# tensorflow/adanet

Hardware: AMD Instinct MI355X
Metric: adanet_iterations_per_hour (higher is better)
Workload: dtype bf16; 1 GPU; model=cifar10-dnn-search (adanet paper space), global_batch=2048, input_dim=3072, n_classes=10, hidden=2048, candidates_per_iter=2, train_steps_per_iter=150, eval_batches=8, parallelism=round_robin1, final_ensemble_size=12

## Files before the change

### adanet_amd/csrc/binding.cpp

```cpp

#include <torch/extension.h>

void gemm_nt_bf16(const at::Tensor& A, const at::Tensor& B, at::Tensor& C,
                  const c10::optional<at::Tensor>& bias, int64_t act,
                  double dropout_p, const c10::optional<at::Tensor>& seed);
void gemm_nt_bf16_probe(const at::Tensor& A, const at::Tensor& B,
                        at::Tensor& C, int64_t variant);
void gemm_nt8(const at::Tensor& A, const at::Tensor& B, at::Tensor& C,
              const c10::optional<at::Tensor>& bias, int64_t act,
              int64_t variant);
void gemm_x8(const at::Tensor& A, const at::Tensor& B, at::Tensor& C,
             const c10::optional<at::Tensor>& bias, int64_t act,
             int64_t trans_a, int64_t trans_b, int64_t variant);
void probe_tr16_layout(at::Tensor& out);
void gemm_tr_probe(const at::Tensor& A, const at::Tensor& B, at::Tensor& C,
                   int64_t trans_a, int64_t trans_b, int64_t variant);
void gemm_tr_bf16(const at::Tensor& A, const at::Tensor& B, at::Tensor& C,
                  const c10::optional<at::Tensor>& bias, int64_t act,
                  int64_t trans_a, int64_t trans_b);
void gemm_tr_batched(const at::Tensor& A, const at::Tensor& B, at::Tensor& C,
                     const c10::optional<at::Tensor>& bias, int64_t act,
                     int64_t trans_a, int64_t trans_b);
void transpose_bf16(const at::Tensor& in, at::Tensor& out);
void softmax_xent_fwd(const at::Tensor& logits, const at::Tensor& labels,
                      const c10::optional<at::Tensor>& loss,
                      at::Tensor& probs, double eps,
                      const c10::optional<at::Tensor>& mean_out);
void softmax_xent_bwd(const at::Tensor& probs, const at::Tensor& labels,
                      const c10::optional<at::Tensor>& grad_rows,
                      at::Tensor& dlogits, double eps,
                      const c10::optional<at::Tensor>& grad_scalar);
void mixer_bwd_dlogits(const at::Tensor& dY, const at::Tensor& weights,
                       at::Tensor& dL, int64_t j, int64_t vector_mode);
void mixer_fwd_direct(const std::vector<at::Tensor>& members,
                      const at::Tensor& weights,
                      const c10::optional<at::Tensor>& bias, at::Tensor& out,
                      int64_t vector_mode);
void mixer_bwd_dw_direct(const std::vector<at::Tensor>& members,
                         const at::Tensor& dY, at::Tensor& dw,
                         int64_t vector_mode);
void fused_sgd(at::Tensor& master, at::Tensor& param, const at::Tensor& grad,
               const c10::optional<at::Tensor>& momentum_buf, double lr,
               double momentum, double dampening, double weight_decay,
               bool nesterov, double grad_scale);
void fused_adam(at::Tensor& master, at::Tensor& param, const at::Tensor& grad,
                at::Tensor& m_buf, at::Tensor& v_buf, double lr, double beta1,
                double beta2, double eps, double weight_decay, int64_t step,
                double grad_scale);
void fused_sgd_fp32(at::Tensor& param, const at::Tensor& grad,
                    const c10::optional<at::Tensor>& momentum_buf, double lr,
                    double momentum, double dampening, double weight_decay,
                    bool nesterov, double grad_scale);
void fused_adam_fp32(at::Tensor& param, const at::Tensor& grad,
                     at::Tensor& m_buf, at::Tensor& v_buf, double lr,
                     double beta1, double beta2, double eps,
                     double weight_decay, int64_t step, double grad_scale);
void layernorm_fwd(const at::Tensor& x, const c10::optional<at::Tensor>& gamma,
                   const c10::optional<at::Tensor>& beta, at::Tensor& y,
                   at::Tensor& mean, at::Tensor& rstd, double eps);
void layernorm_bwd(const at::Tensor& x, const at::Tensor& dy,
                   const c10::optional<at::Tensor>& gamma,
                   const at::Tensor& mean, const at::Tensor& rstd,
                   at::Tensor& dx, const c10::optional<at::Tensor>& dgamma,
                   const c10::optional<at::Tensor>& dbeta);
void dropout_fwd(const at::Tensor& x, at::Tensor& y, double p,
                 const at::Tensor& seed);
void dropout_bwd(const at::Tensor& dy, at::Tensor& dx, double p,
                 const at::Tensor& seed);
void relu_bwd(const at::Tensor& dy, const at::Tensor& y, at::Tensor& dx,
              double scale);
void relu_bwd_colsum(const at::Tensor& dy, const at::Tensor& y,
                     at::Tensor& dz, at::Tensor& db, double scale);
void multi_copy_bf16(const std::vector<at::Tensor>& srcs,
                     const std::vector<at::Tensor>& dsts);
void cell_combine_fwd(const std::vector<at::Tensor>& lefts,
                      const std::vector<at::Tensor>& rights,
                      const std::vector<at::Tensor>& scales_l,
                      const std::vector<at::Tensor>& scales_r, at::Tensor& out,
                      int64_t block_offset);
void cell_combine_bwd(const at::Tensor& dy,
                      const std::vector<at::Tensor>& scales_l,
                      const std::vector<at::Tensor>& scales_r,
                      const std::vector<c10::optional<at::Tensor>>& dlefts,
                      const std::vector<c10::optional<at::Tensor>>& drights,
                      int64_t block_offset);
void augment_draw(const at::Tensor& labels, at::Tensor& params,
                  at::Tensor& labels_out, uint64_t seed, int64_t step,
                  int64_t rank, int64_t world, int64_t N, int64_t pad,
                  int64_t H, int64_t W, bool augment);
void augment_apply(const at::Tensor& data, const at::Tensor& params,
                   const at::Tensor& scale, const at::Tensor& shift,
                   at::Tensor& out, int64_t pad, int64_t cutout_pad);
void colsum_bf16(const at::Tensor& x, at::Tensor& out, int64_t accum);
void binary_histogram(const at::Tensor& scores, const at::Tensor& labels,
                      at::Tensor& hist);
void metrics_multiclass_update(at::Tensor& state, const at::Tensor& logits,
                               const at::Tensor& labels, int64_t k,
                               double eps, bool per_class);
void metrics_binary_update(at::Tensor& state, const at::Tensor& logits,
                           const at::Tensor& labels, int64_t T);
void metrics_regression_update(at::Tensor& state, const at::Tensor& logits,
                               const at::Tensor& labels);
int64_t metrics_max_blocks();
void depthwise_fwd(const at::Tensor& x, const at::Tensor& w, at::Tensor& y,
                   int64_t stride, int64_t pad);
void depthwise_bwd_dx(const at::Tensor& dy, const at::Tensor& w,
                      at::Tensor& dx, int64_t stride, int64_t pad);
void depthwise_bwd_dw(const at::Tensor& x, const at::Tensor& dy,
                      at::Tensor& dw, int64_t stride, int64_t pad);
void argmax_correct(const at::Tensor& logits, const at::Tensor& labels,
                    const c10::optional<at::Tensor>& pred, at::Tensor& correct);
void im2col_bf16(const at::Tensor& x, at::Tensor& out, int64_t K,
                 int64_t stride, int64_t pad);
void col2im_bf16(const at::Tensor& du, at::Tensor& dx, int64_t K,
                 int64_t stride, int64_t pad);
void pool3_fwd(const at::Tensor& x, at::Tensor& y,
               const c10::optional<at::Tensor>& argmax, int64_t stride,
               int64_t is_max);
void pool3_bwd(const at::Tensor& dy, const c10::optional<at::Tensor>& argmax,
               at::Tensor& dx, int64_t stride, int64_t is_max);
void batchnorm_stats(const at::Tensor& x, at::Tensor& mean, at::Tensor& rstd,
                     const c10::optional<at::Tensor>& running_mean,
                     const c10::optional<at::Tensor>& running_var,
                     double eps, double momentum);
void batchnorm_norm(const at::Tensor& x, at::Tensor& y,
                    const at::Tensor& mean, const at::Tensor& rstd,
                    const c10::optional<at::Tensor>& gamma,
                    const c10::optional<at::Tensor>& beta);
void batchnorm_bwd(const at::Tensor& x, const at::Tensor& dy, at::Tensor& dx,
                   const at::Tensor& mean, const at::Tensor& rstd,
                   const c10::optional<at::Tensor>& gamma, at::Tensor& sdy,
                   at::Tensor& sdyx);

PYBIND11_MODULE(TORCH_EXTENSION_NAME, m) {
  m.doc() = "adanet_amd gfx950 (MI355X/CDNA4) kernels";
  m.def("gemm_nt_bf16", &gemm_nt_bf16,
        "C[M,N] = A[M,K] @ B[N,K]^T, fused bias/relu/dropout",
        py::arg("A"), py::arg("B"), py::arg("C"), py::arg("bias"),
        py::arg("act"), py::arg("dropout_p") = 0.0,
        py::arg("seed") = c10::nullopt);
  m.def("gemm_nt_bf16_probe", &gemm_nt_bf16_probe);
  m.def("gemm_nt8", &gemm_nt8,
        "8-phase deep-pipelined GEMM (256^2-class tiles)");
  m.def("gemm_x8", &gemm_x8,
        "pipelined GEMM with K-major (transposed) operand staging");
  m.def("probe_tr16_layout", &probe_tr16_layout);
  m.def("gemm_tr_probe", &gemm_tr_probe);
  m.def("gemm_tr_bf16", &gemm_tr_bf16);
  m.def("gemm_tr_batched", &gemm_tr_batched);
  m.def("transpose_bf16", &transpose_bf16, "bf16 2-D transpose");
  m.def("softmax_xent_fwd", &softmax_xent_fwd);
  m.def("softmax_xent_bwd", &softmax_xent_bwd);
  m.def("mixer_bwd_dlogits", &mixer_bwd_dlogits);
  m.def("mixer_fwd_direct", &mixer_fwd_direct);
  m.def("mixer_bwd_dw_direct", &mixer_bwd_dw_direct);
  m.def("fused_sgd", &fused_sgd);
  m.def("fused_adam", &fused_adam);
  m.def("fused_sgd_fp32", &fused_sgd_fp32);
  m.def("fused_adam_fp32", &fused_adam_fp32);
  m.def("layernorm_fwd", &layernorm_fwd);
  m.def("layernorm_bwd", &layernorm_bwd);
  m.def("dropout_fwd", &dropout_fwd);
  m.def("dropout_bwd", &dropout_bwd);
  m.def("relu_bwd", &relu_bwd, py::arg("dy"), py::arg("y"), py::arg("dx"),
        py::arg("scale") = 1.0);
  m.def("relu_bwd_colsum", &relu_bwd_colsum, py::arg("dy"), py::arg("y"),
        py::arg("dz"), py::arg("db"), py::arg("scale") = 1.0);
  m.def("multi_copy_bf16", &multi_copy_bf16);
  m.def("cell_combine_fwd", &cell_combine_fwd,
        "fused drop-path scale + add + channel concat of up to 8 block pairs",
        py::arg("lefts"), py::arg("rights"), py::arg("scales_l"),
        py::arg("scales_r"), py::arg("out"), py::arg("block_offset") = 0);
  m.def("cell_combine_bwd", &cell_combine_bwd, py::arg("dy"),
        py::arg("scales_l"), py::arg("scales_r"), py::arg("dlefts"),
        py::arg("drights"), py::arg("block_offset") = 0);
  m.def("augment_draw", &augment_draw,
        "per-sample (index, oy, ox, flip, cy, cx) from the counter RNG, plus "
        "the gathered labels",
        py::arg("labels"), py::arg("params"), py::arg("labels_out"),
        py::arg("seed"), py::arg("step"), py::arg("rank"), py::arg("world"),
        py::arg("N"), py::arg("pad"), py::arg("H"), py::arg("W"),
        py::arg("augment") = true);
  m.def("augment_apply", &augment_apply,
        "fused gather + pad-crop + flip + cutout + normalise + bf16 cast",
        py::arg("data"), py::arg("params"), py::arg("scale"),
        py::arg("shift"), py::arg("out"), py::arg("pad"),
        py::arg("cutout_pad"));
  m.def("colsum_bf16", &colsum_bf16, py::arg("x"), py::arg("out"),
        py::arg("accum") = 0);
  m.def("argmax_correct", &argmax_correct);
  m.def("binary_histogram", &binary_histogram);
  m.def("metrics_multiclass_update", &metrics_multiclass_update,
        "streaming loss / top-1 / top-k / per-class counts into an fp64 state",
        py::arg("state"), py::arg("logits"), py::arg("labels"), py::arg("k"),
        py::arg("eps"), py::arg("per_class"));
  m.def("metrics_binary_update", &metrics_binary_update,
        "streaming sigmoid loss / accuracy / [2,T] score histogram",
        py::arg("state"), py::arg("logits"), py::arg("labels"), py::arg("T"));
  m.def("metrics_regression_update", &metrics_regression_update,
        "streaming squared / absolute error sums", py::arg("state"),
        py::arg("logits"), py::arg("labels"));
  m.def("metrics_max_blocks", &metrics_max_blocks,
        "grid cap of the streaming-metric update kernels");
  m.def("im2col_bf16", &im2col_bf16);
  m.def("col2im_bf16", &col2im_bf16);
  m.def("pool3_fwd", &pool3_fwd);
  m.def("pool3_bwd", &pool3_bwd);
  m.def("batchnorm_stats", &batchnorm_stats);
  m.def("batchnorm_norm", &batchnorm_norm);
  m.def("batchnorm_bwd", &batchnorm_bwd);
  m.def("depthwise_fwd", &depthwise_fwd);
  m.def("depthwise_bwd_dx", &depthwise_bwd_dx);
  m.def("depthwise_bwd_dw", &depthwise_bwd_dw);
}
```

### adanet_amd/csrc/common.h

```cpp
#pragma once

#include <hip/hip_runtime.h>
#include <hip/hip_bf16.h>
#include <cstdint>

#define WAVE 64

using bf16_t = __hip_bfloat16;

typedef __attribute__((ext_vector_type(4))) float f32x4;
typedef __attribute__((ext_vector_type(8))) short s16x8;
typedef __attribute__((ext_vector_type(4))) short s16x4;
typedef __attribute__((ext_vector_type(2))) short s16x2;
typedef __attribute__((ext_vector_type(4))) int i32x4;

__device__ __forceinline__ float bf2f(bf16_t x) { return __bfloat162float(x); }
__device__ __forceinline__ bf16_t f2bf(float x) { return __float2bfloat16(x); }

__device__ __forceinline__ float bits2f(short s) {
  union { unsigned int u; float f; } cvt;
  cvt.u = ((unsigned int)(unsigned short)s) << 16;
  return cvt.f;
}

__device__ __forceinline__ short f2bits(float f) {
  union { unsigned int u; float f; } cvt;
  cvt.f = f;
  unsigned int u = cvt.u;
  unsigned int rounding = 0x7fff + ((u >> 16) & 1);
  return (short)((u + rounding) >> 16);
}

__device__ __forceinline__ float wave_reduce_sum(float v) {
#pragma unroll
  for (int off = 32; off > 0; off >>= 1) v += __shfl_xor(v, off, 64);
  return v;
}

__device__ __forceinline__ float wave_reduce_max(float v) {
#pragma unroll
  for (int off = 32; off > 0; off >>= 1) v = fmaxf(v, __shfl_xor(v, off, 64));
  return v;
}


template <int N, typename Emit>
__device__ __forceinline__ void block_reduce_sum(const float (&acc)[N],
                                                 Emit emit) {
  __shared__ float partial[4];
#pragma unroll
  for (int t = 0; t < N; ++t) {
    const float v = wave_reduce_sum(acc[t]);
    if ((threadIdx.x & 63) == 0) partial[threadIdx.x >> 6] = v;
    __syncthreads();
    if (threadIdx.x == 0)
      emit(t, partial[0] + partial[1] + partial[2] + partial[3]);
    __syncthreads();
  }
}

__device__ __forceinline__ float wave_slot_sum(const float* __restrict__ base,
                                               int64_t stride, int n) {
  float s = 0.f;
  for (int r = threadIdx.x & 63; r < n; r += 64) s += base[r * stride];
  return wave_reduce_sum(s);
}

void launch_colsum_reduce(const float* wsp, float* out, int C, int nchunks,
                          int accum, hipStream_t stream);

__device__ __forceinline__ uint32_t hash_rng(uint64_t seed, uint64_t idx) {
  uint64_t z = seed + 0x9e3779b97f4a7c15ull * (idx + 1);
  z = (z ^ (z >> 30)) * 0xbf58476d1ce4e5b9ull;
  z = (z ^ (z >> 27)) * 0x94d049bb133111ebull;
  return (uint32_t)(z >> 32);
}

#define HIP_CHECK_KERNEL()                                                    \
  do {                                                                        \
    hipError_t e = hipGetLastError();                                         \
    if (e != hipSuccess) {                                                    \
      TORCH_CHECK(false, "HIP kernel launch failed: ", hipGetErrorString(e)); \
    }                                                                         \
  } while (0)
```

### adanet_amd/csrc/elementwise.hip

```cpp

#include <torch/extension.h>
#include <ATen/cuda/CUDAContext.h>
#include "common.h"

__global__ __launch_bounds__(256) void dropout_fwd_kernel(
    const bf16_t* __restrict__ x, bf16_t* __restrict__ y, int64_t n, float p,
    const uint64_t* __restrict__ seed_ptr) {
  const float scale = 1.f / (1.f - p);
  const uint32_t thresh = (uint32_t)(p * 4294967296.0f);
  const uint64_t seed = *seed_ptr;
  const int64_t stride = (int64_t)gridDim.x * blockDim.x;
  for (int64_t i = (int64_t)blockIdx.x * blockDim.x + threadIdx.x; i < n;
       i += stride) {
    const bool drop = hash_rng(seed, (uint64_t)i) < thresh;
    y[i] = drop ? f2bf(0.f) : f2bf(bf2f(x[i]) * scale);
  }
}

__global__ __launch_bounds__(256) void dropout_bwd_kernel(
    const bf16_t* __restrict__ dy, bf16_t* __restrict__ dx, int64_t n, float p,
    const uint64_t* __restrict__ seed_ptr) {
  const float scale = 1.f / (1.f - p);
  const uint32_t thresh = (uint32_t)(p * 4294967296.0f);
  const uint64_t seed = *seed_ptr;
  const int64_t stride = (int64_t)gridDim.x * blockDim.x;
  for (int64_t i = (int64_t)blockIdx.x * blockDim.x + threadIdx.x; i < n;
       i += stride) {
    const bool drop = hash_rng(seed, (uint64_t)i) < thresh;
    dx[i] = drop ? f2bf(0.f) : f2bf(bf2f(dy[i]) * scale);
  }
}

__global__ __launch_bounds__(256) void relu_bwd_kernel(
    const bf16_t* __restrict__ dy, const bf16_t* __restrict__ y,
    bf16_t* __restrict__ dx, int64_t n, float scale) {
  const int64_t stride = (int64_t)gridDim.x * blockDim.x;
  for (int64_t i = (int64_t)blockIdx.x * blockDim.x + threadIdx.x; i < n;
       i += stride) {
    dx[i] = bf2f(y[i]) > 0.f ? f2bf(bf2f(dy[i]) * scale) : f2bf(0.f);
  }
}

__global__ __launch_bounds__(256) void relu_bwd_colsum_kernel(
    const bf16_t* __restrict__ dy, const bf16_t* __restrict__ y,
    bf16_t* __restrict__ dz, float* __restrict__ wsp, int B, int C,
    int rows_per_block, float scale) {
  const int c = blockIdx.x * blockDim.x + threadIdx.x;
  if (c >= C) return;
  const int r0 = blockIdx.y * rows_per_block;
  const int r1 = min(B, r0 + rows_per_block);
  float acc = 0.f;
  for (int b = r0; b < r1; ++b) {
    const int64_t i = (int64_t)b * C + c;
    const float g = bf2f(y[i]) > 0.f ? bf2f(dy[i]) * scale : 0.f;
    dz[i] = f2bf(g);
    acc += g;
  }
  wsp[(int64_t)blockIdx.y * C + c] = acc;
}

struct CopyPtrs {
  const bf16_t* s[8];
  bf16_t* d[8];
  int64_t n[8];
};

typedef __attribute__((ext_vector_type(4))) unsigned int u32x4_c;

__global__ __launch_bounds__(256) void multi_copy_bf16_kernel(CopyPtrs P,
                                                              int npairs) {
  const int seg = blockIdx.y;
  if (seg >= npairs) return;
  const bf16_t* __restrict__ s = P.s[seg];
  bf16_t* __restrict__ d = P.d[seg];
  const int64_t n = P.n[seg];
  const int64_t stride = (int64_t)gridDim.x * blockDim.x * 8;
  for (int64_t i = ((int64_t)blockIdx.x * blockDim.x + threadIdx.x) * 8;
       i < n; i += stride) {
    if (i + 8 <= n) {
      *(u32x4_c*)(d + i) = *(const u32x4_c*)(s + i);
    } else {
      for (int64_t j = i; j < n; ++j) d[j] = s[j];
    }
  }
}

void multi_copy_bf16(const std::vector<at::Tensor>& srcs,
                     const std::vector<at::Tensor>& dsts) {
  TORCH_CHECK(srcs.size() == dsts.size(), "multi_copy: pair count mismatch");
  auto stream = at::cuda::getCurrentCUDAStream();
  for (size_t j0 = 0; j0 < srcs.size(); j0 += 8) {
    const int np = (int)std::min<size_t>(8, srcs.size() - j0);
    CopyPtrs P;
    int64_t maxn = 0;
    for (int k = 0; k < np; ++k) {
      const at::Tensor& s = srcs[j0 + k];
      const at::Tensor& d = dsts[j0 + k];
      TORCH_CHECK(s.is_cuda() && d.is_cuda() &&
                      s.scalar_type() == at::kBFloat16 &&
                      d.scalar_type() == at::kBFloat16 &&
                      s.is_contiguous() && d.is_contiguous() &&
                      s.numel() == d.numel(),
                  "multi_copy: contiguous bf16 same-size pairs required");
      P.s[k] = (const bf16_t*)s.data_ptr();
      P.d[k] = (bf16_t*)d.data_ptr();
      P.n[k] = s.numel();
      maxn = std::max(maxn, P.n[k]);
    }
    if (maxn == 0) continue;
    const int blocks =
        (int)std::min<int64_t>((maxn + 8 * 256 - 1) / (8 * 256), 512);
    hipLaunchKernelGGL(multi_copy_bf16_kernel,
                       dim3((unsigned)blocks, (unsigned)np), dim3(256), 0,
                       stream.stream(), P, np);
    HIP_CHECK_KERNEL();
  }
}

static int ew_grid(int64_t n) {
  return (int)std::min<int64_t>((n + 255) / 256, 2048);
}

void dropout_fwd(const at::Tensor& x, at::Tensor& y, double p,
                 const at::Tensor& seed) {
  const int64_t n = x.numel();
  if (n == 0) return;
  TORCH_CHECK(seed.is_cuda() && seed.scalar_type() == at::kLong,
              "dropout: device int64 seed tensor required");
  auto stream = at::cuda::getCurrentCUDAStream();
  hipLaunchKernelGGL(dropout_fwd_kernel, dim3(ew_grid(n)), dim3(256), 0,
                     stream.stream(), (const bf16_t*)x.data_ptr(),
                     (bf16_t*)y.data_ptr(), n, (float)p,
                     (const uint64_t*)seed.data_ptr());
  HIP_CHECK_KERNEL();
}

void dropout_bwd(const at::Tensor& dy, at::Tensor& dx, double p,
                 const at::Tensor& seed) {
  const int64_t n = dy.numel();
  if (n == 0) return;
  auto stream = at::cuda::getCurrentCUDAStream();
  hipLaunchKernelGGL(dropout_bwd_kernel, dim3(ew_grid(n)), dim3(256), 0,
                     stream.stream(), (const bf16_t*)dy.data_ptr(),
                     (bf16_t*)dx.data_ptr(), n, (float)p,
                     (const uint64_t*)seed.data_ptr());
  HIP_CHECK_KERNEL();
}

void relu_bwd(const at::Tensor& dy, const at::Tensor& y, at::Tensor& dx,
              double scale) {
  const int64_t n = dy.numel();
  if (n == 0) return;
  auto stream = at::cuda::getCurrentCUDAStream();
  hipLaunchKernelGGL(relu_bwd_kernel, dim3(ew_grid(n)), dim3(256), 0,
                     stream.stream(), (const bf16_t*)dy.data_ptr(),
                     (const bf16_t*)y.data_ptr(), (bf16_t*)dx.data_ptr(), n,
                     (float)scale);
  HIP_CHECK_KERNEL();
}

void relu_bwd_colsum(const at::Tensor& dy, const at::Tensor& y,
                     at::Tensor& dz, at::Tensor& db, double scale) {
  TORCH_CHECK(dy.is_contiguous() && y.is_contiguous() && dz.is_contiguous(),
              "relu_bwd_colsum: contiguous tensors required");
  TORCH_CHECK(db.scalar_type() == at::kFloat, "relu_bwd_colsum: fp32 db");
  const int B = (int)dy.size(0), C = (int)dy.size(1);
  if (B == 0 || C == 0) return;
  auto stream = at::cuda::getCurrentCUDAStream();
  const int stripes = (C + 255) / 256;
  const int row_chunks =
      std::max(1, std::min(1024 / stripes, (B + 7) / 8));
  const int rows_per_block = (B + row_chunks - 1) / row_chunks;
  auto wsp = at::empty({row_chunks, C}, db.options());
  hipLaunchKernelGGL(relu_bwd_colsum_kernel,
                     dim3((unsigned)stripes, (unsigned)row_chunks), dim3(256),
                     0, stream.stream(), (const bf16_t*)dy.data_ptr(),
                     (const bf16_t*)y.data_ptr(), (bf16_t*)dz.data_ptr(),
                     wsp.data_ptr<float>(), B, C, rows_per_block,
                     (float)scale);
  launch_colsum_reduce(wsp.data_ptr<float>(), db.data_ptr<float>(), C,
                       row_chunks, 1, stream.stream());
  HIP_CHECK_KERNEL();
}
```

### adanet_amd/csrc/gemm_8ph.hip

```cpp

#include <torch/extension.h>
#include <ATen/cuda/CUDAContext.h>
#include "common.h"

namespace {

template <int HROWS>
__device__ __forceinline__ void stage_half(
    const bf16_t* __restrict__ G, int64_t ld, int rows0, int max_row, int k0,
    bf16_t* __restrict__ lds_half, int wid, int lane) {
#pragma unroll
  for (int r = 0; r < HROWS / 64; ++r) {
    const int row_in_half = r * 64 + wid * 8 + (lane >> 3);
    int grow = rows0 + row_in_half;
    grow = grow < max_row ? grow : max_row - 1;
    const int src_blk = (lane & 7) ^ ((lane >> 3) & 7);
    const bf16_t* gp = G + (int64_t)grow * ld + k0 + src_blk * 8;
    bf16_t* lp = lds_half + (r * 64 + wid * 8) * 64;
    __builtin_amdgcn_global_load_lds(
        (const __attribute__((address_space(1))) void*)gp,
        (__attribute__((address_space(3))) void*)lp, 16, 0, 0);
  }
}

__device__ __forceinline__ s16x8 lds_frag(const bf16_t* lds, int row,
                                          int blk8) {
  const int pblk = blk8 ^ (row & 7);
  const uint32_t addr = (uint32_t)(uintptr_t)(
      const __attribute__((address_space(3))) void*)&lds[row * 64 + pblk * 8];
  s16x8 out;
  asm volatile("ds_read_b128 %0, %1" : "=v"(out) : "v"(addr));
  return out;
}

#define S_BARRIER() __builtin_amdgcn_s_barrier()

template <int N>
__device__ __forceinline__ void vmcnt_wait() {
  static_assert((N >= 0 && N <= 4) || N == 6 || N == 8,
                "unsupported vmcnt");
  if constexpr (N == 6) {
    asm volatile("s_waitcnt vmcnt(6)" ::: "memory");
    return;
  }
  if constexpr (N == 8) {
    asm volatile("s_waitcnt vmcnt(8)" ::: "memory");
    return;
  }
  if constexpr (N == 0) {
    asm volatile("s_waitcnt vmcnt(0)" ::: "memory");
  } else if constexpr (N == 1) {
    asm volatile("s_waitcnt vmcnt(1)" ::: "memory");
  } else if constexpr (N == 2) {
    asm volatile("s_waitcnt vmcnt(2)" ::: "memory");
  } else if constexpr (N == 3) {
    asm volatile("s_waitcnt vmcnt(3)" ::: "memory");
  } else if constexpr (N == 4) {
    asm volatile("s_waitcnt vmcnt(4)" ::: "memory");
  }
}

template <int BM, int BN, bool SAFE = false, bool SETPRIO = true>
__global__ __launch_bounds__(512, 2) void gemm_nt8_kernel(
    const bf16_t* __restrict__ A, const bf16_t* __restrict__ B,
    bf16_t* __restrict__ C, const float* __restrict__ bias, int M, int N,
    int K, int64_t lda, int64_t ldb, int64_t ldc, int act, int mtiles,
    int ntiles, const long long* __restrict__ seed = nullptr,
    uint32_t pthresh = 0, float inv_keep = 1.f) {
  constexpr int FM = BM / (2 * 16);
  constexpr int FN = BN / (4 * 16);
  constexpr int MG = FM / 4;
  static_assert(FM >= 4, "need >=1 m-rep per phase");
  constexpr int HA = BM / 2;
  constexpr int HB = BN / 2;
  constexpr int LB = HB / 64;
  __shared__ bf16_t As[2][BM * 64];
  __shared__ bf16_t Bs[2][BN * 64];

  const int nwg = mtiles * ntiles;
  const int orig = blockIdx.x;
  const int q = nwg >> 3, r = nwg & 7, xcd = orig & 7;
  const int wg = (xcd < r ? xcd * (q + 1) : r * (q + 1) + (xcd - r) * q) +
                 (orig >> 3);
  const int tile_m = wg / ntiles, tile_n = wg % ntiles;
  const int row0 = tile_m * BM, col0 = tile_n * BN;

  const int tid = threadIdx.x;
  const int wid = tid >> 6, lane = tid & 63;
  const int wm = wid >> 2, wn = wid & 3;

  f32x4 acc[FM][FN];
#pragma unroll
  for (int i = 0; i < FM; ++i)
#pragma unroll
    for (int j = 0; j < FN; ++j) acc[i][j] = f32x4{0.f, 0.f, 0.f, 0.f};

  const int NT = K / 64;

  stage_half<HA>(A, lda, row0, M, 0, &As[0][0], wid, lane);
  stage_half<HA>(A, lda, row0 + HA, M, 0, &As[0][HA * 64], wid, lane);
  stage_half<HB>(B, ldb, col0, N, 0, &Bs[0][0], wid, lane);
  stage_half<HB>(B, ldb, col0 + HB, N, 0, &Bs[0][HB * 64], wid, lane);
  if (NT > 1) {
    stage_half<HB>(B, ldb, col0, N, 64, &Bs[1][0], wid, lane);
    stage_half<HB>(B, ldb, col0 + HB, N, 64, &Bs[1][HB * 64], wid, lane);
    if (SAFE) vmcnt_wait<0>(); else vmcnt_wait<2 * LB>();
  } else {
    vmcnt_wait<0>();
  }
  S_BARRIER();

  const int arow_base = wm * (FM * 16) + (lane & 15);
  const int brow_base = wn * (FN * 16) + (lane & 15);
  const int kblk = (lane >> 4);

  for (int t = 0; t < NT; ++t) {
    const int buf = t & 1;
    const bf16_t* at = &As[buf][0];
    const bf16_t* bt = &Bs[buf][0];
    s16x8 bfrag[FN][2];
#pragma unroll
    for (int p = 0; p < 4; ++p) {
      s16x8 afrag[MG][2];
#pragma unroll
      for (int g = 0; g < MG; ++g) {
        const int m = p * MG + g;
#pragma unroll
        for (int kk = 0; kk < 2; ++kk)
          afrag[g][kk] =
              lds_frag(at, arow_base + m * 16, kk * 4 + kblk);
      }
      if (p == 0) {
#pragma unroll
        for (int n = 0; n < FN; ++n)
#pragma unroll
          for (int kk = 0; kk < 2; ++kk)
            bfrag[n][kk] =
                lds_frag(bt, brow_base + n * 16, kk * 4 + kblk);
      }
      if (p == 0 && t + 1 < NT) {
        stage_half<HA>(A, lda, row0, M, (t + 1) * 64, &As[buf ^ 1][0], wid,
                       lane);
      } else if (p == 1 && t + 1 < NT) {
        stage_half<HA>(A, lda, row0 + HA, M, (t + 1) * 64,
                       &As[buf ^ 1][HA * 64], wid, lane);
      } else if (p == 2 && t + 2 < NT) {
        stage_half<HB>(B, ldb, col0, N, (t + 2) * 64, &Bs[buf][0], wid,
                       lane);
      } else if (p == 3 && t + 2 < NT) {
        stage_half<HB>(B, ldb, col0 + HB, N, (t + 2) * 64,
                       &Bs[buf][HB * 64], wid, lane);
      }
      if (p == 3) {
        if (SAFE) vmcnt_wait<0>(); else vmcnt_wait<2 * LB>();
      }
      if (SAFE) {
        __syncthreads();
      } else {
        S_BARRIER();
      }
      asm volatile("s_waitcnt lgkmcnt(0)" ::: "memory");
      __builtin_amdgcn_sched_barrier(0);
      if (SETPRIO) __builtin_amdgcn_s_setprio(1);
#pragma unroll
      for (int g = 0; g < MG; ++g) {
        const int m = p * MG + g;
#pragma unroll
        for (int n = 0; n < FN; ++n)
#pragma unroll
          for (int kk = 0; kk < 2; ++kk)
            acc[m][n] = __builtin_amdgcn_mfma_f32_16x16x32_bf16(
                afrag[g][kk], bfrag[n][kk], acc[m][n], 0, 0, 0);
      }
      if (SETPRIO) __builtin_amdgcn_s_setprio(0);
      if (SAFE) {
        __syncthreads();
      } else {
        S_BARRIER();
      }
    }
  }

  const int c_col_in_frag = lane & 15;
  const int c_row_base = (lane >> 4) * 4;
#pragma unroll
  for (int i = 0; i < FM; ++i) {
#pragma unroll
    for (int j = 0; j < FN; ++j) {
      const int col = col0 + wn * (FN * 16) + j * 16 + c_col_in_frag;
      if (col >= N) continue;
      const float bv = bias ? bias[col] : 0.f;
#pragma unroll
      for (int rr = 0; rr < 4; ++rr) {
        const int row = row0 + wm * (FM * 16) + i * 16 + c_row_base + rr;
        if (row >= M) continue;
        float v = acc[i][j][rr] + bv;
        if (act == 1) v = v > 0.f ? v : 0.f;
        if (act == 3) {
          v = v > 0.f ? v : 0.f;
          const uint32_t r =
              hash_rng((uint64_t)seed[0], (uint64_t)row * N + col);
          v = (r >= pthresh) ? v * inv_keep : 0.f;
        }
        bf16_t* cp = &C[(int64_t)row * ldc + col];
        if (act == 2) v += bf2f(*cp);
        *cp = f2bf(v);
      }
    }
  }
}

template <int N>
__device__ __forceinline__ void lgkm_wait() {
  static_assert(N == 0 || N == 2 || N == 4, "unsupported lgkmcnt");
  if constexpr (N == 0) {
    asm volatile("s_waitcnt lgkmcnt(0)" ::: "memory");
  } else if constexpr (N == 2) {
    asm volatile("s_waitcnt lgkmcnt(2)" ::: "memory");
  } else if constexpr (N == 4) {
    asm volatile("s_waitcnt lgkmcnt(4)" ::: "memory");
  }
}

template <int BM, int BN, bool SETPRIO = false>
__global__ __launch_bounds__(512, 2) void gemm_nt8p_kernel(
    const bf16_t* __restrict__ A, const bf16_t* __restrict__ B,
    bf16_t* __restrict__ C, const float* __restrict__ bias, int M, int N,
    int K, int64_t lda, int64_t ldb, int64_t ldc, int act, int mtiles,
    int ntiles) {
  constexpr int FM = BM / (2 * 16);
  constexpr int FN = BN / (4 * 16);
  constexpr int MG = FM / 4;
  static_assert(FM >= 4, "need >=1 m-rep per phase");
  constexpr int HA = BM / 2;
  constexpr int HB = BN / 2;
  constexpr int LB = HB / 64;
  __shared__ bf16_t As[2][BM * 64];
  __shared__ bf16_t Bs[2][BN * 64];

  const int nwg = mtiles * ntiles;
  const int orig = blockIdx.x;
  const int q = nwg >> 3, r = nwg & 7, xcd = orig & 7;
  const int wg = (xcd < r ? xcd * (q + 1) : r * (q + 1) + (xcd - r) * q) +
                 (orig >> 3);
  const int tile_m = wg / ntiles, tile_n = wg % ntiles;
  const int row0 = tile_m * BM, col0 = tile_n * BN;

  const int tid = threadIdx.x;
  const int wid = tid >> 6, lane = tid & 63;
  const int wm = wid >> 2, wn = wid & 3;

  f32x4 acc[FM][FN];
#pragma unroll
  for (int i = 0; i < FM; ++i)
#pragma unroll
    for (int j = 0; j < FN; ++j) acc[i][j] = f32x4{0.f, 0.f, 0.f, 0.f};

  const int NT = K / 64;

  stage_half<HA>(A, lda, row0, M, 0, &As[0][0], wid, lane);
  stage_half<HA>(A, lda, row0 + HA, M, 0, &As[0][HA * 64], wid, lane);
  stage_half<HB>(B, ldb, col0, N, 0, &Bs[0][0], wid, lane);
  stage_half<HB>(B, ldb, col0 + HB, N, 0, &Bs[0][HB * 64], wid, lane);
  if (NT > 1) {
    stage_half<HB>(B, ldb, col0, N, 64, &Bs[1][0], wid, lane);
    stage_half<HB>(B, ldb, col0 + HB, N, 64, &Bs[1][HB * 64], wid, lane);
    vmcnt_wait<2 * LB>();
  } else {
    vmcnt_wait<0>();
  }
  S_BARRIER();

  const int arow_base = wm * (FM * 16) + (lane & 15);
  const int brow_base = wn * (FN * 16) + (lane & 15);
  const int kblk = (lane >> 4);

  s16x8 bfrag[FN][2];
  s16x8 afrag[2][MG][2];

  for (int t = 0; t < NT; ++t) {
    const int buf = t & 1;
    const bf16_t* at = &As[buf][0];
    const bf16_t* bt = &Bs[buf][0];
    const bool pre_b0 = t + 2 < NT;

#pragma unroll
    for (int n = 0; n < FN; ++n)
#pragma unroll
      for (int kk = 0; kk < 2; ++kk)
        bfrag[n][kk] = lds_frag(bt, brow_base + n * 16, kk * 4 + kblk);
#pragma unroll
    for (int g = 0; g < MG; ++g)
#pragma unroll
      for (int kk = 0; kk < 2; ++kk)
        afrag[0][g][kk] =
            lds_frag(at, arow_base + g * 16, kk * 4 + kblk);
#pragma unroll
    for (int g = 0; g < MG; ++g)
#pragma unroll
      for (int kk = 0; kk < 2; ++kk)
        afrag[1][g][kk] =
            lds_frag(at, arow_base + (MG + g) * 16, kk * 4 + kblk);
    if (t + 1 < NT)
      stage_half<HA>(A, lda, row0, M, (t + 1) * 64, &As[buf ^ 1][0], wid,
                     lane);
    lgkm_wait<2 * MG>();
    __builtin_amdgcn_sched_barrier(0);
    if (SETPRIO) __builtin_amdgcn_s_setprio(1);
#pragma unroll
    for (int g = 0; g < MG; ++g)
#pragma unroll
      for (int n = 0; n < FN; ++n)
#pragma unroll
        for (int kk = 0; kk < 2; ++kk)
          acc[g][n] = __builtin_amdgcn_mfma_f32_16x16x32_bf16(
              afrag[0][g][kk], bfrag[n][kk], acc[g][n], 0, 0, 0);
    if (SETPRIO) __builtin_amdgcn_s_setprio(0);
    S_BARRIER();

#pragma unroll
    for (int p = 1; p < 3; ++p) {
      const int cur = p & 1, nxt = cur ^ 1;
#pragma unroll
      for (int g = 0; g < MG; ++g)
#pragma unroll
        for (int kk = 0; kk < 2; ++kk)
          afrag[nxt][g][kk] = lds_frag(
              at, arow_base + ((p + 1) * MG + g) * 16, kk * 4 + kblk);
      if (p == 1) {
        if (t + 1 < NT)
          stage_half<HA>(A, lda, row0 + HA, M, (t + 1) * 64,
                         &As[buf ^ 1][HA * 64], wid, lane);
      } else {
        if (pre_b0)
          stage_half<HB>(B, ldb, col0, N, (t + 2) * 64, &Bs[buf][0], wid,
                         lane);
      }
      lgkm_wait<2 * MG>();
      __builtin_amdgcn_sched_barrier(0);
      if (SETPRIO) __builtin_amdgcn_s_setprio(1);
#pragma unroll
      for (int g = 0; g < MG; ++g)
#pragma unroll
        for (int n = 0; n < FN; ++n)
#pragma unroll
          for (int kk = 0; kk < 2; ++kk)
            acc[p * MG + g][n] = __builtin_amdgcn_mfma_f32_16x16x32_bf16(
                afrag[cur][g][kk], bfrag[n][kk], acc[p * MG + g][n], 0, 0,
                0);
      if (SETPRIO) __builtin_amdgcn_s_setprio(0);
      S_BARRIER();
    }

    if (pre_b0) {
      vmcnt_wait<LB>();
    } else {
      vmcnt_wait<0>();
    }
    if (t + 2 < NT)
      stage_half<HB>(B, ldb, col0 + HB, N, (t + 2) * 64, &Bs[buf][HB * 64],
                     wid, lane);
    lgkm_wait<0>();
    __builtin_amdgcn_sched_barrier(0);
    if (SETPRIO) __builtin_amdgcn_s_setprio(1);
#pragma unroll
    for (int g = 0; g < MG; ++g)
#pragma unroll
      for (int n = 0; n < FN; ++n)
#pragma unroll
        for (int kk = 0; kk < 2; ++kk)
          acc[3 * MG + g][n] = __builtin_amdgcn_mfma_f32_16x16x32_bf16(
              afrag[1][g][kk], bfrag[n][kk], acc[3 * MG + g][n], 0, 0, 0);
    if (SETPRIO) __builtin_amdgcn_s_setprio(0);
    S_BARRIER();
  }

  const int c_col_in_frag = lane & 15;
  const int c_row_base = (lane >> 4) * 4;
#pragma unroll
  for (int i = 0; i < FM; ++i) {
#pragma unroll
    for (int j = 0; j < FN; ++j) {
      const int col = col0 + wn * (FN * 16) + j * 16 + c_col_in_frag;
      if (col >= N) continue;
      const float bv = bias ? bias[col] : 0.f;
#pragma unroll
      for (int rr = 0; rr < 4; ++rr) {
        const int row = row0 + wm * (FM * 16) + i * 16 + c_row_base + rr;
        if (row >= M) continue;
        float v = acc[i][j][rr] + bv;
        if (act == 1) v = v > 0.f ? v : 0.f;
        bf16_t* cp = &C[(int64_t)row * ldc + col];
        if (act == 2) v += bf2f(*cp);
        *cp = f2bf(v);
      }
    }
  }
}


template <int ROWS, int NW>
__device__ __forceinline__ void stage_slab(
    const bf16_t* __restrict__ G, int64_t ld, int rows0, int max_row, int k0,
    bf16_t* __restrict__ lds_slab, int wid, int lane) {
#pragma unroll
  for (int r = 0; r < ROWS / (NW * 16); ++r) {
    const int row_in = r * (NW * 16) + wid * 16 + (lane >> 2);
    int grow = rows0 + row_in;
    grow = grow < max_row ? grow : max_row - 1;
    const int src_blk = (lane & 3) ^ ((lane >> 3) & 3);
    const bf16_t* gp = G + (int64_t)grow * ld + k0 + src_blk * 8;
    bf16_t* lp = lds_slab + (r * (NW * 16) + wid * 16) * 32;
    __builtin_amdgcn_global_load_lds(
        (const __attribute__((address_space(1))) void*)gp,
        (__attribute__((address_space(3))) void*)lp, 16, 0, 0);
  }
}

typedef __attribute__((ext_vector_type(2))) unsigned int u32x2_k;

__device__ __forceinline__ u32x2_k ks_tr_read(const bf16_t* p) {
  const unsigned off = (unsigned)(uintptr_t)(
      const __attribute__((address_space(3))) bf16_t*)p;
  u32x2_k out;
  asm volatile("ds_read_b64_tr_b16 %0, %1" : "=v"(out) : "v"(off));
  return out;
}

template <int COLS, int NW>
__device__ __forceinline__ void stage_slab_tr(
    const bf16_t* __restrict__ G, int64_t ld, int col0, int max_col, int k0,
    int max_k, bf16_t* __restrict__ lds_slab, int wid, int lane) {
  constexpr int SUBT = COLS / 16;
#pragma unroll
  for (int st = wid; st < SUBT; st += NW) {
    const int k = k0 + (lane >> 1);
    int col = col0 + st * 16 + (lane & 1) * 8;
    if (col + 8 > max_col) col = max(0, (max_col - 8) & ~7);
    const bf16_t* gp = G + (int64_t)min(k, max_k - 1) * ld + col;
    bf16_t* lp = lds_slab + st * 512;
    __builtin_amdgcn_global_load_lds(
        (const __attribute__((address_space(1))) void*)gp,
        (__attribute__((address_space(3))) void*)lp, 16, 0, 0);
  }
}

__device__ __forceinline__ s16x8 lds_frag_ks_tr(const bf16_t* lds_slab,
                                                int colblock, int lane) {
  const bf16_t* sub = lds_slab + colblock * 512;
  const int row = 8 * (lane >> 4) + ((lane >> 2) & 3);
  const int col4 = 4 * (lane & 3);
  u32x2_k r0 = ks_tr_read(sub + row * 16 + col4);
  u32x2_k r1 = ks_tr_read(sub + (row + 4) * 16 + col4);
  union {
    s16x8 f;
    struct { u32x2_k lo, hi; } u;
  } pack;
  pack.u.lo = r0;
  pack.u.hi = r1;
  return pack.f;
}

__device__ __forceinline__ s16x8 lds_frag_ks(const bf16_t* lds_slab,
                                             int row, int q) {
  const int blk = q ^ ((row >> 1) & 3);
  const uint32_t addr = (uint32_t)(uintptr_t)(
      const __attribute__((address_space(3))) void*)
      &lds_slab[row * 32 + blk * 8];
  s16x8 out;
  asm volatile("ds_read_b128 %0, %1" : "=v"(out) : "v"(addr));
  return out;
}

template <int BM, int BN, int WN, bool TRA = false, bool TRB = false,
          bool BAR2 = false,
          bool STAGGER = false>
__global__ __launch_bounds__(2 * WN * 64, 2) void gemm_ks_kernel(
    const bf16_t* __restrict__ A, const bf16_t* __restrict__ B,
    bf16_t* __restrict__ C, const float* __restrict__ bias, int M, int N,
    int K, int64_t lda, int64_t ldb, int64_t ldc, int act, int mtiles,
    int ntiles, const long long* __restrict__ seed = nullptr,
    uint32_t pthresh = 0, float inv_keep = 1.f) {
  constexpr int NW = 2 * WN;
  constexpr int FM = BM / 32;
  constexpr int FN = BN / (WN * 16);
  constexpr int MH = FM / 2;
  static_assert(FM >= 2, "need >=1 m-rep per phase pair");
  constexpr int LPU_A = BM / (NW * 16);
  constexpr int LPU_B = BN / (NW * 16);
  constexpr int INFLIGHT = 2 * LPU_A + 2 * LPU_B;
  __shared__ bf16_t As[2][2][BM * 32];
  __shared__ bf16_t Bs[2][2][BN * 32];

  const int nwg = mtiles * ntiles;
  const int orig = blockIdx.x;
  const int q = nwg >> 3, r = nwg & 7, xcd = orig & 7;
  const int wg = (xcd < r ? xcd * (q + 1) : r * (q + 1) + (xcd - r) * q) +
                 (orig >> 3);
  const int tile_m = wg / ntiles, tile_n = wg % ntiles;
  const int row0 = tile_m * BM, col0 = tile_n * BN;

  const int tid = threadIdx.x;
  const int wid = tid >> 6, lane = tid & 63;
  const int wm = wid / WN, wn = wid % WN;

  f32x4 acc[FM][FN];
#pragma unroll
  for (int i = 0; i < FM; ++i)
#pragma unroll
    for (int j = 0; j < FN; ++j) acc[i][j] = f32x4{0.f, 0.f, 0.f, 0.f};

  if (STAGGER && (wid & 1) == 0) __builtin_amdgcn_s_setprio(1);

  const int NT = K / 64;

#define KS_STAGE_A(buf, slab, t_)                                             \
  do {                                                                        \
    if (TRA)                                                                  \
      stage_slab_tr<BM, NW>(A, lda, row0, M, (t_)*64 + (slab)*32, K,          \
                            &As[buf][slab][0], wid, lane);                    \
    else                                                                      \
      stage_slab<BM, NW>(A, lda, row0, M, (t_)*64 + (slab)*32,                \
                         &As[buf][slab][0], wid, lane);                       \
  } while (0)
#define KS_STAGE_B(buf, slab, t_)                                             \
  do {                                                                        \
    if (TRB)                                                                  \
      stage_slab_tr<BN, NW>(B, ldb, col0, N, (t_)*64 + (slab)*32, K,          \
                            &Bs[buf][slab][0], wid, lane);                    \
    else                                                                      \
      stage_slab<BN, NW>(B, ldb, col0, N, (t_)*64 + (slab)*32,                \
                         &Bs[buf][slab][0], wid, lane);                       \
  } while (0)

  KS_STAGE_A(0, 0, 0);
  KS_STAGE_B(0, 0, 0);
  KS_STAGE_A(0, 1, 0);
  KS_STAGE_B(0, 1, 0);
  if (NT > 1) {
    KS_STAGE_A(1, 0, 1);
    KS_STAGE_B(1, 0, 1);
    vmcnt_wait<INFLIGHT>();
  } else {
    vmcnt_wait<0>();
  }
  S_BARRIER();

  const int arow_base = wm * (FM * 16) + (lane & 15);
  const int brow_base = wn * (FN * 16) + (lane & 15);
  const int kq = lane >> 4;

  for (int t = 0; t < NT; ++t) {
    const int buf = t & 1;
#pragma unroll
    for (int kk = 0; kk < 2; ++kk) {
      const bf16_t* at = &As[buf][kk][0];
      const bf16_t* bt = &Bs[buf][kk][0];
      s16x8 bfrag[FN];
#pragma unroll
      for (int ph = 0; ph < 2; ++ph) {
        s16x8 afrag[MH];
        if (ph == 0) {
#pragma unroll
          for (int n = 0; n < FN; ++n)
            bfrag[n] = TRB ? lds_frag_ks_tr(bt, wn * FN + n, lane)
                           : lds_frag_ks(bt, brow_base + n * 16, kq);
        }
#pragma unroll
        for (int g = 0; g < MH; ++g)
          afrag[g] = TRA
              ? lds_frag_ks_tr(at, wm * FM + ph * MH + g, lane)
              : lds_frag_ks(at, arow_base + (ph * MH + g) * 16, kq);
        if (kk == 0) {
          const int tn = t + 1 < NT ? t + 1 : NT - 1;
          if (ph == 0) {
            KS_STAGE_A(buf ^ 1, 1, tn);
          } else {
            KS_STAGE_B(buf ^ 1, 1, tn);
          }
        } else {
          const int tn = t + 2 < NT ? t + 2 : NT - 1;
          if (ph == 0) {
            KS_STAGE_A(buf, 0, tn);
          } else {
            KS_STAGE_B(buf, 0, tn);
          }
        }
        asm volatile("s_waitcnt lgkmcnt(0)" ::: "memory");
        __builtin_amdgcn_sched_barrier(0);
#pragma unroll
        for (int g = 0; g < MH; ++g)
#pragma unroll
          for (int n = 0; n < FN; ++n)
            acc[ph * MH + g][n] = __builtin_amdgcn_mfma_f32_16x16x32_bf16(
                afrag[g], bfrag[n], acc[ph * MH + g][n], 0, 0, 0);
        if (ph == 1) {
          vmcnt_wait<INFLIGHT>();
          S_BARRIER();
        } else if (BAR2) {
          S_BARRIER();
        }
      }
    }
  }
#undef KS_STAGE_A
#undef KS_STAGE_B

  const int c_col_in_frag = lane & 15;
  const int c_row_base = (lane >> 4) * 4;
#pragma unroll
  for (int i = 0; i < FM; ++i) {
#pragma unroll
    for (int j = 0; j < FN; ++j) {
      const int col = col0 + wn * (FN * 16) + j * 16 + c_col_in_frag;
      if (col >= N) continue;
      const float bv = bias ? bias[col] : 0.f;
#pragma unroll
      for (int rr = 0; rr < 4; ++rr) {
        const int row = row0 + wm * (FM * 16) + i * 16 + c_row_base + rr;
        if (row >= M) continue;
        float v = acc[i][j][rr] + bv;
        if (act == 1) v = v > 0.f ? v : 0.f;
        if (act == 3) {
          v = v > 0.f ? v : 0.f;
          const uint32_t rnd =
              hash_rng((uint64_t)seed[0], (uint64_t)row * N + col);
          v = (rnd >= pthresh) ? v * inv_keep : 0.f;
        }
        bf16_t* cp = &C[(int64_t)row * ldc + col];
        if (act == 2) v += bf2f(*cp);
        *cp = f2bf(v);
      }
    }
  }
}

}


typedef __attribute__((ext_vector_type(2))) unsigned int u32x2_g;

__device__ __forceinline__ u32x2_g tr8_b16_read(const bf16_t* p) {
  const unsigned off = (unsigned)(uintptr_t)(
      const __attribute__((address_space(3))) bf16_t*)p;
  u32x2_g out;
  asm volatile("ds_read_b64_tr_b16 %0, %1" : "=v"(out) : "v"(off));
  return out;
}

namespace {

template <int HROWS, int NW>
__device__ __forceinline__ void stage_half_g(
    const bf16_t* __restrict__ G, int64_t ld, int rows0, int max_row, int k0,
    bf16_t* __restrict__ lds_half, int wid, int lane) {
#pragma unroll
  for (int r = 0; r < HROWS / (NW * 8); ++r) {
    const int row_in_half = r * (NW * 8) + wid * 8 + (lane >> 3);
    int grow = rows0 + row_in_half;
    grow = grow < max_row ? grow : max_row - 1;
    const int src_blk = (lane & 7) ^ ((lane >> 3) & 7);
    const bf16_t* gp = G + (int64_t)grow * ld + k0 + src_blk * 8;
    bf16_t* lp = lds_half + (r * (NW * 8) + wid * 8) * 64;
    __builtin_amdgcn_global_load_lds(
        (const __attribute__((address_space(1))) void*)gp,
        (__attribute__((address_space(3))) void*)lp, 16, 0, 0);
  }
}

template <int HCOLS, int NW>
__device__ __forceinline__ void stage_half_tr8(
    const bf16_t* __restrict__ G, int64_t ld, int col0, int max_col, int k0,
    int max_k, bf16_t* __restrict__ lds_half, int wid, int lane) {
  constexpr int SUBT = HCOLS / 16;
#pragma unroll
  for (int slab = 0; slab < 2; ++slab) {
#pragma unroll
    for (int st = wid; st < SUBT; st += NW) {
      const int k = k0 + slab * 32 + (lane >> 1);
      int col = col0 + st * 16 + (lane & 1) * 8;
      if (col + 8 > max_col) col = max(0, (max_col - 8) & ~7);
      const bf16_t* gp = G + (int64_t)min(k, max_k - 1) * ld + col;
      bf16_t* lp = lds_half + slab * HCOLS * 32 + st * 512;
      __builtin_amdgcn_global_load_lds(
          (const __attribute__((address_space(1))) void*)gp,
          (__attribute__((address_space(3))) void*)lp, 16, 0, 0);
    }
  }
}

template <int HCOLS>
__device__ __forceinline__ s16x8 frag_tr8(const bf16_t* lds_half,
                                          int colblock, int kk, int lane) {
  const bf16_t* sub = lds_half + kk * HCOLS * 32 + colblock * 512;
  const int row = 8 * (lane >> 4) + ((lane >> 2) & 3);
  const int col4 = 4 * (lane & 3);
  u32x2_g r0 = tr8_b16_read(sub + row * 16 + col4);
  u32x2_g r1 = tr8_b16_read(sub + (row + 4) * 16 + col4);
  union {
    s16x8 f;
    struct { u32x2_g lo, hi; } u;
  } pack;
  pack.u.lo = r0;
  pack.u.hi = r1;
  return pack.f;
}

template <int N>
__device__ __forceinline__ void lgkm_wait_g() {
  static_assert(N == 0 || N == 2 || N == 4 || N == 8, "lgkm count");
  if constexpr (N == 0) asm volatile("s_waitcnt lgkmcnt(0)" ::: "memory");
  else if constexpr (N == 2) asm volatile("s_waitcnt lgkmcnt(2)" ::: "memory");
  else if constexpr (N == 4) asm volatile("s_waitcnt lgkmcnt(4)" ::: "memory");
  else if constexpr (N == 8) asm volatile("s_waitcnt lgkmcnt(8)" ::: "memory");
}

template <int BM, int BN, int WN, bool TRA, bool TRB>
__global__ __launch_bounds__(2 * WN * 64, 2) void gemm_x8_kernel(
    const bf16_t* __restrict__ A, const bf16_t* __restrict__ B,
    bf16_t* __restrict__ C, const float* __restrict__ bias, int M, int N,
    int K, int64_t lda, int64_t ldb, int64_t ldc, int act, int mtiles,
    int ntiles) {
  constexpr int NW = 2 * WN;
  constexpr int FM = BM / (2 * 16);
  constexpr int FN = BN / (WN * 16);
  constexpr int MG = FM / 4;
  static_assert(FM >= 4, "need >=1 m-rep per phase");
  constexpr int HA = BM / 2;
  constexpr int HB = BN / 2;
  constexpr int LB = HB / (8 * NW) > 0 ? HB / (8 * NW) : 1;
  __shared__ bf16_t As[2][BM * 64];
  __shared__ bf16_t Bs[2][BN * 64];

  const int nwg = mtiles * ntiles;
  const int orig = blockIdx.x;
  const int q = nwg >> 3, r = nwg & 7, xcd = orig & 7;
  const int wg = (xcd < r ? xcd * (q + 1) : r * (q + 1) + (xcd - r) * q) +
                 (orig >> 3);
  const int tile_m = wg / ntiles, tile_n = wg % ntiles;
  const int row0 = tile_m * BM, col0 = tile_n * BN;

  const int tid = threadIdx.x;
  const int wid = tid >> 6, lane = tid & 63;
  const int wm = wid / WN, wn = wid % WN;

  f32x4 acc[FM][FN];
#pragma unroll
  for (int i = 0; i < FM; ++i)
#pragma unroll
    for (int j = 0; j < FN; ++j) acc[i][j] = f32x4{0.f, 0.f, 0.f, 0.f};

  const int NT = K / 64;

#define STAGE_A8(buf, half, k0)                                               \
  do {                                                                        \
    if (TRA)                                                                  \
      stage_half_tr8<HA, NW>(A, lda, row0 + (half)*HA, M, k0, K,              \
                             &As[buf][(half)*HA * 64], wid, lane);            \
    else                                                                      \
      stage_half_g<HA, NW>(A, lda, row0 + (half)*HA, M, k0,                   \
                           &As[buf][(half)*HA * 64], wid, lane);              \
  } while (0)
#define STAGE_B8(buf, half, k0)                                               \
  do {                                                                        \
    if (TRB)                                                                  \
      stage_half_tr8<HB, NW>(B, ldb, col0 + (half)*HB, N, k0, K,              \
                             &Bs[buf][(half)*HB * 64], wid, lane);            \
    else                                                                      \
      stage_half_g<HB, NW>(B, ldb, col0 + (half)*HB, N, k0,                   \
                           &Bs[buf][(half)*HB * 64], wid, lane);              \
  } while (0)

  STAGE_A8(0, 0, 0);
  STAGE_A8(0, 1, 0);
  STAGE_B8(0, 0, 0);
  STAGE_B8(0, 1, 0);
  if (NT > 1) {
    STAGE_B8(1, 0, 64);
    STAGE_B8(1, 1, 64);
    vmcnt_wait<2 * LB>();
  } else {
    vmcnt_wait<0>();
  }
  S_BARRIER();

  const int arow_base = wm * (FM * 16) + (lane & 15);
  const int brow_base = wn * (FN * 16) + (lane & 15);
  const int kblk = (lane >> 4);

#define LOAD_A8(dst, at_, m)                                                  \
  do {                                                                        \
    if (TRA) {                                                                \
      const int cb = (wm * FM + (m)) % (HA / 16);                             \
      const bf16_t* hbase = (at_) + ((wm * FM + (m)) / (HA / 16)) * HA * 64;  \
      (dst)[0] = frag_tr8<HA>(hbase, cb, 0, lane);                            \
      (dst)[1] = frag_tr8<HA>(hbase, cb, 1, lane);                            \
    } else {                                                                  \
      (dst)[0] = lds_frag(at_, arow_base + (m)*16, kblk);                     \
      (dst)[1] = lds_frag(at_, arow_base + (m)*16, 4 + kblk);                 \
    }                                                                         \
  } while (0)
#define LOAD_B8(dst, bt_, n)                                                  \
  do {                                                                        \
    if (TRB) {                                                                \
      const int cb = (wn * FN + (n)) % (HB / 16);                             \
      const bf16_t* hbase = (bt_) + ((wn * FN + (n)) / (HB / 16)) * HB * 64;  \
      (dst)[0] = frag_tr8<HB>(hbase, cb, 0, lane);                            \
      (dst)[1] = frag_tr8<HB>(hbase, cb, 1, lane);                            \
    } else {                                                                  \
      (dst)[0] = lds_frag(bt_, brow_base + (n)*16, kblk);                     \
      (dst)[1] = lds_frag(bt_, brow_base + (n)*16, 4 + kblk);                 \
    }                                                                         \
  } while (0)

  s16x8 bfrag[FN][2];
  s16x8 afrag[2][MG][2];
  constexpr int AG_READS = MG * 2 * (TRA ? 2 : 1);

  for (int t = 0; t < NT; ++t) {
    const int buf = t & 1;
    const bf16_t* at = &As[buf][0];
    const bf16_t* bt = &Bs[buf][0];
    const bool pre_b0 = t + 2 < NT;

#pragma unroll
    for (int n = 0; n < FN; ++n) LOAD_B8(bfrag[n], bt, n);
#pragma unroll
    for (int g = 0; g < MG; ++g) LOAD_A8(afrag[0][g], at, g);
#pragma unroll
    for (int g = 0; g < MG; ++g) LOAD_A8(afrag[1][g], at, MG + g);
    if (t + 1 < NT) STAGE_A8(buf ^ 1, 0, (t + 1) * 64);
    lgkm_wait_g<AG_READS>();
    __builtin_amdgcn_sched_barrier(0);
#pragma unroll
    for (int g = 0; g < MG; ++g)
#pragma unroll
      for (int n = 0; n < FN; ++n)
#pragma unroll
        for (int kk = 0; kk < 2; ++kk)
          acc[g][n] = __builtin_amdgcn_mfma_f32_16x16x32_bf16(
              afrag[0][g][kk], bfrag[n][kk], acc[g][n], 0, 0, 0);
    S_BARRIER();

#pragma unroll
    for (int p = 1; p < 3; ++p) {
      const int cur = p & 1, nxt = cur ^ 1;
#pragma unroll
      for (int g = 0; g < MG; ++g)
        LOAD_A8(afrag[nxt][g], at, (p + 1) * MG + g);
      if (p == 1) {
        if (t + 1 < NT) STAGE_A8(buf ^ 1, 1, (t + 1) * 64);
      } else {
        if (pre_b0) STAGE_B8(buf, 0, (t + 2) * 64);
      }
      lgkm_wait_g<AG_READS>();
      __builtin_amdgcn_sched_barrier(0);
#pragma unroll
      for (int g = 0; g < MG; ++g)
#pragma unroll
        for (int n = 0; n < FN; ++n)
#pragma unroll
          for (int kk = 0; kk < 2; ++kk)
            acc[p * MG + g][n] = __builtin_amdgcn_mfma_f32_16x16x32_bf16(
                afrag[cur][g][kk], bfrag[n][kk], acc[p * MG + g][n], 0, 0,
                0);
      S_BARRIER();
    }

    if (pre_b0) {
      vmcnt_wait<LB>();
    } else {
      vmcnt_wait<0>();
    }
    if (t + 2 < NT) STAGE_B8(buf, 1, (t + 2) * 64);
    lgkm_wait_g<0>();
    __builtin_amdgcn_sched_barrier(0);
#pragma unroll
    for (int g = 0; g < MG; ++g)
#pragma unroll
      for (int n = 0; n < FN; ++n)
#pragma unroll
        for (int kk = 0; kk < 2; ++kk)
          acc[3 * MG + g][n] = __builtin_amdgcn_mfma_f32_16x16x32_bf16(
              afrag[1][g][kk], bfrag[n][kk], acc[3 * MG + g][n], 0, 0, 0);
    S_BARRIER();
  }
#undef STAGE_A8
#undef STAGE_B8
#undef LOAD_A8
#undef LOAD_B8

  const int c_col_in_frag = lane & 15;
  const int c_row_base = (lane >> 4) * 4;
#pragma unroll
  for (int i = 0; i < FM; ++i) {
#pragma unroll
    for (int j = 0; j < FN; ++j) {
      const int col = col0 + wn * (FN * 16) + j * 16 + c_col_in_frag;
      if (col >= N) continue;
      const float bv = bias ? bias[col] : 0.f;
#pragma unroll
      for (int rr = 0; rr < 4; ++rr) {
        const int row = row0 + wm * (FM * 16) + i * 16 + c_row_base + rr;
        if (row >= M) continue;
        float v = acc[i][j][rr] + bv;
        if (act == 1) v = v > 0.f ? v : 0.f;
        bf16_t* cp = &C[(int64_t)row * ldc + col];
        if (act == 2) v += bf2f(*cp);
        *cp = f2bf(v);
      }
    }
  }
}

}

void gemm_x8(const at::Tensor& A, const at::Tensor& B, at::Tensor& C,
             const c10::optional<at::Tensor>& bias, int64_t act,
             int64_t trans_a, int64_t trans_b, int64_t variant) {
  const int M = (int)C.size(0), N = (int)C.size(1);
  const int K = (int)(trans_a ? A.size(0) : A.size(1));
  TORCH_CHECK((int)(trans_b ? B.size(1) : B.size(0)) == N &&
              (int)(trans_b ? B.size(0) : B.size(1)) == K &&
              (int)(trans_a ? A.size(1) : A.size(0)) == M,
              "gemm_x8: shape mismatch");
  TORCH_CHECK(K % 64 == 0, "gemm_x8: K % 64");
  const int64_t lda = A.stride(0), ldb = B.stride(0), ldc = C.stride(0);
  TORCH_CHECK(lda % 8 == 0 && ldb % 8 == 0, "gemm_x8: 16B-aligned rows");
  const float* bias_ptr = nullptr;
  if (bias.has_value() && bias->defined()) bias_ptr = bias->data_ptr<float>();
  auto stream = at::cuda::getCurrentCUDAStream();
  const bf16_t* a = (const bf16_t*)A.data_ptr();
  const bf16_t* b = (const bf16_t*)B.data_ptr();
  bf16_t* c = (bf16_t*)C.data_ptr();

#define LX8(BM, BN, WNW, TA, TB)                                              \
  do {                                                                        \
    const int mt = (M + BM - 1) / BM, nt = (N + BN - 1) / BN;                 \
    hipLaunchKernelGGL((gemm_x8_kernel<BM, BN, WNW, TA, TB>), dim3(mt * nt),  \
                       dim3(2 * WNW * 64), 0, stream.stream(), a, b, c,       \
                       bias_ptr, M, N, K, lda, ldb, ldc, (int)act, mt, nt);   \
  } while (0)
#define LX8_T(BM, BN, WNW)                                                    \
  do {                                                                        \
    if (trans_a && trans_b) LX8(BM, BN, WNW, true, true);                     \
    else if (trans_b) LX8(BM, BN, WNW, false, true);                          \
    else if (trans_a) LX8(BM, BN, WNW, true, false);                          \
    else LX8(BM, BN, WNW, false, false);                                      \
  } while (0)
  switch (variant) {
    case 0: LX8_T(128, 128, 4); break;
    case 1: LX8_T(128, 128, 2); break;
    case 2: LX8_T(256, 256, 4); break;
    case 3: LX8_T(256, 128, 4); break;
    case 4: LX8_T(128, 256, 4); break;
#define LKS_T(BM, BN, WNW)                                                    \
  do {                                                                        \
    const int mt = (M + BM - 1) / BM, nt = (N + BN - 1) / BN;                 \
    if (trans_a && trans_b) {                                                 \
      hipLaunchKernelGGL((gemm_ks_kernel<BM, BN, WNW, true, true>),           \
                         dim3(mt * nt), dim3(2 * WNW * 64), 0,                \
                         stream.stream(), a, b, c, bias_ptr, M, N, K, lda,    \
                         ldb, ldc, (int)act, mt, nt);                         \
    } else if (trans_b) {                                                     \
      hipLaunchKernelGGL((gemm_ks_kernel<BM, BN, WNW, false, true>),          \
                         dim3(mt * nt), dim3(2 * WNW * 64), 0,                \
                         stream.stream(), a, b, c, bias_ptr, M, N, K, lda,    \
                         ldb, ldc, (int)act, mt, nt);                         \
    } else if (trans_a) {                                                     \
      hipLaunchKernelGGL((gemm_ks_kernel<BM, BN, WNW, true, false>),          \
                         dim3(mt * nt), dim3(2 * WNW * 64), 0,                \
                         stream.stream(), a, b, c, bias_ptr, M, N, K, lda,    \
                         ldb, ldc, (int)act, mt, nt);                         \
    } else {                                                                  \
      hipLaunchKernelGGL((gemm_ks_kernel<BM, BN, WNW, false, false>),         \
                         dim3(mt * nt), dim3(2 * WNW * 64), 0,                \
                         stream.stream(), a, b, c, bias_ptr, M, N, K, lda,    \
                         ldb, ldc, (int)act, mt, nt);                         \
    }                                                                         \
  } while (0)
    case 10: LKS_T(128, 128, 4); break;
    case 11: LKS_T(256, 256, 4); break;
    case 12: LKS_T(256, 128, 4); break;
#undef LKS_T
    default: TORCH_CHECK(false, "gemm_x8: unknown variant");
  }
#undef LX8
#undef LX8_T
  HIP_CHECK_KERNEL();
}

bool gemm_nt8_try(const bf16_t* a, const bf16_t* b, bf16_t* c,
                  const float* bias_ptr, int M, int N, int K, int64_t lda,
                  int64_t ldb, int64_t ldc, int act, hipStream_t stream) {
  if (K % 64 != 0 || K < 128 || lda % 8 || ldb % 8) return false;
  const int64_t t256 = (int64_t)((M + 255) / 256) * ((N + 255) / 256);
  const int64_t t128 = (int64_t)((M + 127) / 128) * ((N + 127) / 128);
  if (t256 >= 200) {
    const int mt = (M + 255) / 256, nt = (N + 255) / 256;
    hipLaunchKernelGGL((gemm_nt8_kernel<256, 256, false, false>),
                       dim3(mt * nt), dim3(512), 0, stream, a, b, c,
                       bias_ptr, M, N, K, lda, ldb, ldc, act, mt, nt);
    return true;
  }
  if (t128 >= 256) {
    const int mt = (M + 127) / 128, nt = (N + 127) / 128;
    hipLaunchKernelGGL((gemm_ks_kernel<128, 128, 4>), dim3(mt * nt),
                       dim3(512), 0, stream, a, b, c, bias_ptr, M, N, K,
                       lda, ldb, ldc, act, mt, nt);
    return true;
  }
  return false;
}

bool gemm_nt8_try_dropout(const bf16_t* a, const bf16_t* b, bf16_t* c,
                          const float* bias_ptr, int M, int N, int K,
                          int64_t lda, int64_t ldb, int64_t ldc,
                          const long long* seed, uint32_t pthresh,
                          float inv_keep, hipStream_t stream) {
  if (K % 64 != 0 || K < 128 || lda % 8 || ldb % 8) return false;
  const int64_t t256 = (int64_t)((M + 255) / 256) * ((N + 255) / 256);
  const int64_t t128 = (int64_t)((M + 127) / 128) * ((N + 127) / 128);
  if (t256 >= 200) {
    const int mt = (M + 255) / 256, nt = (N + 255) / 256;
    hipLaunchKernelGGL((gemm_nt8_kernel<256, 256, false, false>),
                       dim3(mt * nt), dim3(512), 0, stream, a, b, c,
                       bias_ptr, M, N, K, lda, ldb, ldc, 3, mt, nt, seed,
                       pthresh, inv_keep);
    return true;
  }
  if (t128 >= 256) {
    const int mt = (M + 127) / 128, nt = (N + 127) / 128;
    hipLaunchKernelGGL((gemm_ks_kernel<128, 128, 4>), dim3(mt * nt),
                       dim3(512), 0, stream, a, b, c, bias_ptr, M, N, K,
                       lda, ldb, ldc, 3, mt, nt, seed, pthresh, inv_keep);
    return true;
  }
  return false;
}

void gemm_nt8(const at::Tensor& A, const at::Tensor& B, at::Tensor& C,
              const c10::optional<at::Tensor>& bias, int64_t act,
              int64_t variant) {
  TORCH_CHECK(A.is_cuda() && B.is_cuda() && C.is_cuda(), "gemm8: GPU only");
  TORCH_CHECK(A.scalar_type() == at::kBFloat16 &&
              B.scalar_type() == at::kBFloat16, "gemm8: bf16 inputs");
  const int M = (int)A.size(0), K = (int)A.size(1), N = (int)B.size(0);
  TORCH_CHECK(B.size(1) == K && C.size(0) == M && C.size(1) == N,
              "gemm8: shape mismatch");
  TORCH_CHECK(K % 64 == 0, "gemm8: K % 64 != 0");
  const int64_t lda = A.stride(0), ldb = B.stride(0), ldc = C.stride(0);
  TORCH_CHECK(A.stride(1) == 1 && B.stride(1) == 1 && C.stride(1) == 1 &&
              lda % 8 == 0 && ldb % 8 == 0, "gemm8: need 16B-aligned rows");
  const float* bias_ptr = nullptr;
  if (bias.has_value() && bias->defined()) {
    TORCH_CHECK(bias->scalar_type() == at::kFloat && bias->numel() == N,
                "gemm8: bias must be fp32[N]");
    bias_ptr = bias->data_ptr<float>();
  }
  auto stream = at::cuda::getCurrentCUDAStream();
  const bf16_t* a = (const bf16_t*)A.data_ptr();
  const bf16_t* b = (const bf16_t*)B.data_ptr();
  bf16_t* c = (bf16_t*)C.data_ptr();

#define LAUNCH_8PH(BM, BN, SAFE, PRIO)                                        \
  do {                                                                        \
    const int mt = (M + BM - 1) / BM, nt = (N + BN - 1) / BN;                 \
    hipLaunchKernelGGL((gemm_nt8_kernel<BM, BN, SAFE, PRIO>), dim3(mt * nt),  \
                       dim3(512), 0, stream.stream(), a, b, c, bias_ptr, M,   \
                       N, K, lda, ldb, ldc, (int)act, mt, nt);                \
  } while (0)

  switch (variant) {
    case 0: LAUNCH_8PH(256, 256, false, true); break;
    case 1: LAUNCH_8PH(256, 128, false, true); break;
    case 2: LAUNCH_8PH(128, 256, false, true); break;
    case 3: LAUNCH_8PH(128, 128, false, true); break;
    case 10: LAUNCH_8PH(256, 256, true, true); break;
    case 11: LAUNCH_8PH(256, 128, true, true); break;
    case 12: LAUNCH_8PH(128, 256, true, true); break;
    case 13: LAUNCH_8PH(128, 128, true, true); break;
    case 20: LAUNCH_8PH(256, 256, false, false); break;
    case 23: LAUNCH_8PH(128, 128, false, false); break;
#define LAUNCH_8PHP(BM, BN, PRIO)                                             \
  do {                                                                        \
    const int mt = (M + BM - 1) / BM, nt = (N + BN - 1) / BN;                 \
    hipLaunchKernelGGL((gemm_nt8p_kernel<BM, BN, PRIO>), dim3(mt * nt),       \
                       dim3(512), 0, stream.stream(), a, b, c, bias_ptr, M,   \
                       N, K, lda, ldb, ldc, (int)act, mt, nt);                \
  } while (0)
#define LAUNCH_KS(BM, BN, WNW)                                               \
  do {                                                                        \
    const int mt = (M + BM - 1) / BM, nt = (N + BN - 1) / BN;                 \
    hipLaunchKernelGGL((gemm_ks_kernel<BM, BN, WNW>), dim3(mt * nt),          \
                       dim3(2 * WNW * 64), 0, stream.stream(), a, b, c,       \
                       bias_ptr, M, N, K, lda, ldb, ldc, (int)act, mt, nt);   \
  } while (0)
    case 50: LAUNCH_KS(256, 256, 4); break;
    case 51: LAUNCH_KS(128, 128, 4); break;
    case 52: LAUNCH_KS(128, 128, 2); break;
    case 53: LAUNCH_KS(256, 128, 4); break;
    case 55: {
      const int mt = (M + 255) / 256, nt = (N + 255) / 256;
      hipLaunchKernelGGL(
          (gemm_ks_kernel<256, 256, 4, false, false, false>), dim3(mt * nt),
          dim3(512), 0, stream.stream(), a, b, c, bias_ptr, M, N, K, lda,
          ldb, ldc, (int)act, mt, nt);
      break;
    }
    case 56: {
      const int mt = (M + 127) / 128, nt = (N + 127) / 128;
      hipLaunchKernelGGL(
          (gemm_ks_kernel<128, 128, 4, false, false, false>), dim3(mt * nt),
          dim3(512), 0, stream.stream(), a, b, c, bias_ptr, M, N, K, lda,
          ldb, ldc, (int)act, mt, nt);
      break;
    }
    case 57: {
      const int mt = (M + 255) / 256, nt = (N + 255) / 256;
      hipLaunchKernelGGL(
          (gemm_ks_kernel<256, 256, 4, false, false, false, true>),
          dim3(mt * nt), dim3(512), 0, stream.stream(), a, b, c, bias_ptr,
          M, N, K, lda, ldb, ldc, (int)act, mt, nt);
      break;
    }
    case 58: {
      const int mt = (M + 127) / 128, nt = (N + 127) / 128;
      hipLaunchKernelGGL(
          (gemm_ks_kernel<128, 128, 4, false, false, false, true>),
          dim3(mt * nt), dim3(512), 0, stream.stream(), a, b, c, bias_ptr,
          M, N, K, lda, ldb, ldc, (int)act, mt, nt);
      break;
    }
#undef LAUNCH_KS
    case 30: LAUNCH_8PHP(256, 256, false); break;
    case 31: LAUNCH_8PHP(256, 256, true); break;
    case 32: LAUNCH_8PHP(256, 128, false); break;
    case 33: LAUNCH_8PHP(128, 256, false); break;
    case 34: LAUNCH_8PHP(128, 128, false); break;
#undef LAUNCH_8PHP
    default: TORCH_CHECK(false, "gemm8: unknown variant");
  }
#undef LAUNCH_8PH
  HIP_CHECK_KERNEL();
}
```

### adanet_amd/csrc/gemm_tn.hip

```cpp

#include <torch/extension.h>
#include <ATen/cuda/CUDAContext.h>
#include "common.h"

typedef s16x8 frag_ab;
typedef __attribute__((ext_vector_type(2))) unsigned int u32x2;

void gemm_x8(const at::Tensor& A, const at::Tensor& B, at::Tensor& C,
             const c10::optional<at::Tensor>& bias, int64_t act,
             int64_t trans_a, int64_t trans_b, int64_t variant);

typedef __attribute__((address_space(3))) const bf16_t* lds_cptr_t;

__device__ __forceinline__ u32x2 tr_b16_read(const bf16_t* lds_half_addr) {
  const unsigned off = (unsigned)(uintptr_t)(lds_cptr_t)lds_half_addr;
  u32x2 out;
  asm volatile("ds_read_b64_tr_b16 %0, %1"
               : "=v"(out)
               : "v"(off)
               : "memory");
  return out;
}

__device__ __forceinline__ void tr_frag_addrs(const bf16_t* sub, int lane,
                                              const bf16_t** a1,
                                              const bf16_t** a2) {
  const int row = 8 * (lane >> 4) + ((lane >> 2) & 3);
  const int col4 = 4 * (lane & 3);
  *a1 = sub + row * 16 + col4;
  *a2 = sub + (row + 4) * 16 + col4;
}

__global__ void probe_tr16_layout_kernel(float* __restrict__ out) {
  __shared__ bf16_t tile[32 * 16];
  const int lane = threadIdx.x & 63;
  for (int i = threadIdx.x; i < 32 * 16; i += blockDim.x) {
    tile[i] = f2bf((float)(i % 256));
  }
  __syncthreads();
  const bf16_t *a1, *a2;
  tr_frag_addrs(tile, lane, &a1, &a2);
  u32x2 r0 = tr_b16_read(a1);
  u32x2 r1 = tr_b16_read(a2);
  asm volatile("s_waitcnt lgkmcnt(0)" ::: "memory");
  __builtin_amdgcn_sched_barrier(0);
  const unsigned short* h0 = (const unsigned short*)&r0;
  const unsigned short* h1 = (const unsigned short*)&r1;
  if (blockIdx.x == 0) {
#pragma unroll
    for (int j = 0; j < 4; ++j) {
      const unsigned short a = h0[j];
      const unsigned short b = h1[j];
      out[lane * 8 + j] = bits2f(*(const short*)&a);
      out[lane * 8 + 4 + j] = bits2f(*(const short*)&b);
    }
  }
}

void probe_tr16_layout(at::Tensor& out) {
  auto stream = at::cuda::getCurrentCUDAStream();
  hipLaunchKernelGGL(probe_tr16_layout_kernel, dim3(1), dim3(64), 0,
                     stream.stream(), out.data_ptr<float>());
  HIP_CHECK_KERNEL();
}

template <int ROWS, int NWAVES>
__device__ __forceinline__ void stage_tile_tr(
    const bf16_t* __restrict__ G, int ld, int tile_col0, int max_col, int k0,
    int max_k, bf16_t* __restrict__ lds, int wid, int lane) {
  constexpr int SUBTILES = ROWS / 16;
#pragma unroll
  for (int st = wid; st < SUBTILES; st += NWAVES) {
    const int k = k0 + (lane >> 1);
    int col = tile_col0 + st * 16 + (lane & 1) * 8;
    if (col + 8 > max_col) {
      col = max(0, (max_col - 8) & ~7);
    }
    const bf16_t* gp = G + (int64_t)min(k, max_k - 1) * ld + col;
    bf16_t* lp = lds + st * 32 * 16;
    __builtin_amdgcn_global_load_lds(
        (const __attribute__((address_space(1))) void*)gp,
        (__attribute__((address_space(3))) void*)lp, 16, 0, 0);
  }
}

__device__ __forceinline__ frag_ab frag_from_tr(const bf16_t* lds,
                                                int row_block, int lane) {
  const bf16_t* sub = lds + row_block * 32 * 16;
  const bf16_t *a1, *a2;
  tr_frag_addrs(sub, lane, &a1, &a2);
  u32x2 r0 = tr_b16_read(a1);
  u32x2 r1 = tr_b16_read(a2);
  union {
    frag_ab f;
    struct { u32x2 lo, hi; } u;
  } pack;
  pack.u.lo = r0;
  pack.u.hi = r1;
  return pack.f;
}

template <int BM, int BN, int FM, int FN, int MINWAVES, int WGM, int WGN,
          bool TRA, bool TRB, int GROUPM = 0>
__global__ __launch_bounds__(WGM * WGN * 64, MINWAVES) void gemm_tr_kernel(
    const bf16_t* __restrict__ A, const bf16_t* __restrict__ B,
    bf16_t* __restrict__ C, const float* __restrict__ bias, int M, int N,
    int K, int lda, int ldb, int ldc, int act, int mtiles, int ntiles,
    int64_t stride_a = 0, int64_t stride_b = 0, int64_t stride_c = 0) {
  constexpr int KSTEP = 32;
  __shared__ bf16_t As[2][BM * KSTEP];
  __shared__ bf16_t Bs[2][BN * KSTEP];
  A += (int64_t)blockIdx.z * stride_a;
  B += (int64_t)blockIdx.z * stride_b;
  C += (int64_t)blockIdx.z * stride_c;
  const int nwg = mtiles * ntiles;
  const int orig = blockIdx.x;
  const int q = nwg >> 3, r = nwg & 7, xcd = orig & 7;
  const int wg = (xcd < r ? xcd * (q + 1) : r * (q + 1) + (xcd - r) * q) +
                 (orig >> 3);
  int tile_m, tile_n;
  if (GROUPM > 0) {
    const int per_band = GROUPM * ntiles;
    const int band = wg / per_band;
    const int in_band = wg % per_band;
    const int gm = min(GROUPM, mtiles - band * GROUPM);
    tile_m = band * GROUPM + in_band % gm;
    tile_n = in_band / gm;
  } else {
    tile_m = wg / ntiles;
    tile_n = wg % ntiles;
  }
  static_assert(BM == WGM * FM * 16 && BN == WGN * FN * 16, "geometry");
  constexpr int NWAVES = WGM * WGN;
  const int tid = threadIdx.x;
  const int wid = tid >> 6;
  const int lane = tid & 63;
  const int wm = wid / WGN, wn = wid % WGN;
  const int row0 = tile_m * BM;
  const int col0 = tile_n * BN;

  f32x4 acc[FM][FN];
#pragma unroll
  for (int i = 0; i < FM; ++i)
#pragma unroll
    for (int j = 0; j < FN; ++j) acc[i][j] = f32x4{0.f, 0.f, 0.f, 0.f};

  const int ktiles = K / KSTEP;

#define STAGE_A(buf, k0)                                                      \
  do {                                                                        \
    if (TRA)                                                                  \
      stage_tile_tr<BM, NWAVES>(A, lda, row0, M, k0, K, As[buf], wid, lane);  \
    else {                                                                    \
      constexpr int RPS = 512 / KSTEP;                                        \
      constexpr int LPR = KSTEP / 8;                                          \
      for (int seg = wid; seg < BM / RPS; seg += NWAVES) {                    \
        const int rt = seg * RPS + lane / LPR;                                \
        int grow = row0 + rt;                                                 \
        grow = grow < M ? grow : M - 1;                                       \
        const bf16_t* gp = A + (int64_t)grow * lda + k0 + (lane % LPR) * 8;   \
        bf16_t* lp = As[buf] + seg * RPS * KSTEP;                             \
        __builtin_amdgcn_global_load_lds(                                     \
            (const __attribute__((address_space(1))) void*)gp,                \
            (__attribute__((address_space(3))) void*)lp, 16, 0, 0);           \
      }                                                                       \
    }                                                                         \
  } while (0)
#define STAGE_B(buf, k0)                                                      \
  do {                                                                        \
    if (TRB)                                                                  \
      stage_tile_tr<BN, NWAVES>(B, ldb, col0, N, k0, K, Bs[buf], wid, lane);  \
    else {                                                                    \
      constexpr int RPS = 512 / KSTEP;                                        \
      constexpr int LPR = KSTEP / 8;                                          \
      for (int seg = wid; seg < BN / RPS; seg += NWAVES) {                    \
        const int rt = seg * RPS + lane / LPR;                                \
        int grow = col0 + rt;                                                 \
        grow = grow < N ? grow : N - 1;                                       \
        const bf16_t* gp = B + (int64_t)grow * ldb + k0 + (lane % LPR) * 8;   \
        bf16_t* lp = Bs[buf] + seg * RPS * KSTEP;                             \
        __builtin_amdgcn_global_load_lds(                                     \
            (const __attribute__((address_space(1))) void*)gp,                \
            (__attribute__((address_space(3))) void*)lp, 16, 0, 0);           \
      }                                                                       \
    }                                                                         \
  } while (0)

  STAGE_A(0, 0);
  STAGE_B(0, 0);
  int buf = 0;
  for (int kt = 0; kt < ktiles; ++kt) {
    asm volatile("s_waitcnt vmcnt(0)" ::: "memory");
    __syncthreads();
    if (kt + 1 < ktiles) {
      STAGE_A(buf ^ 1, (kt + 1) * KSTEP);
      STAGE_B(buf ^ 1, (kt + 1) * KSTEP);
    }
    frag_ab a[FM], b[FN];
    const int kofs = (lane >> 4) * 8;
#pragma unroll
    for (int f = 0; f < FM; ++f) {
      if (TRA) {
        a[f] = frag_from_tr(As[buf], wm * FM + f, lane);
      } else {
        const int arow = wm * (FM * 16) + (lane & 15);
        a[f] = *(const frag_ab*)&As[buf][(arow + f * 16) * KSTEP + kofs];
      }
    }
#pragma unroll
    for (int f = 0; f < FN; ++f) {
      if (TRB) {
        b[f] = frag_from_tr(Bs[buf], wn * FN + f, lane);
      } else {
        const int brow = wn * (FN * 16) + (lane & 15);
        b[f] = *(const frag_ab*)&Bs[buf][(brow + f * 16) * KSTEP + kofs];
      }
    }
    if (TRA || TRB) {
      asm volatile("s_waitcnt lgkmcnt(0)" ::: "memory");
      __builtin_amdgcn_sched_barrier(0);
    }
#pragma unroll
    for (int i = 0; i < FM; ++i)
#pragma unroll
      for (int j = 0; j < FN; ++j)
        acc[i][j] = __builtin_amdgcn_mfma_f32_16x16x32_bf16(a[i], b[j],
                                                            acc[i][j], 0, 0,
                                                            0);
    buf ^= 1;
  }

  const int c_col_in_frag = lane & 15;
  const int c_row_base = (lane >> 4) * 4;
#pragma unroll
  for (int i = 0; i < FM; ++i) {
#pragma unroll
    for (int j = 0; j < FN; ++j) {
      const int col = col0 + wn * (FN * 16) + j * 16 + c_col_in_frag;
      if (col >= N) continue;
      const float bv = bias ? bias[col] : 0.f;
#pragma unroll
      for (int rr = 0; rr < 4; ++rr) {
        const int row = row0 + wm * (FM * 16) + i * 16 + c_row_base + rr;
        if (row >= M) continue;
        float v = acc[i][j][rr] + bv;
        if (act == 1) v = v > 0.f ? v : 0.f;
        bf16_t* cp = &C[(int64_t)row * ldc + col];
        if (act == 2) v += bf2f(*cp);
        *cp = f2bf(v);
      }
    }
  }
#undef STAGE_A
#undef STAGE_B
}

void gemm_tr_probe(const at::Tensor& A, const at::Tensor& B, at::Tensor& C,
                   int64_t trans_a, int64_t trans_b, int64_t variant) {
  const int M = (int)C.size(0), N = (int)C.size(1);
  const int K = (int)(trans_a ? A.size(0) : A.size(1));
  const int lda = (int)A.stride(0), ldb = (int)B.stride(0),
            ldc = (int)C.stride(0);
  auto stream = at::cuda::getCurrentCUDAStream();
  const bf16_t* a = (const bf16_t*)A.data_ptr();
  const bf16_t* b = (const bf16_t*)B.data_ptr();
  bf16_t* c = (bf16_t*)C.data_ptr();
#define LV(BM, BN, FM, FN, MW, WGM, WGN, GM)                                  \
  do {                                                                        \
    const int mt = (M + BM - 1) / BM, nt = (N + BN - 1) / BN;                 \
    if (trans_a && trans_b) {                                                 \
      hipLaunchKernelGGL(                                                     \
          (gemm_tr_kernel<BM, BN, FM, FN, MW, WGM, WGN, true, true, GM>),     \
          dim3(mt * nt), dim3(WGM * WGN * 64), 0, stream.stream(), a, b, c,  \
          nullptr, M, N, K, lda, ldb, ldc, 0, mt, nt);                        \
    } else if (trans_b) {                                                     \
      hipLaunchKernelGGL(                                                     \
          (gemm_tr_kernel<BM, BN, FM, FN, MW, WGM, WGN, false, true, GM>),    \
          dim3(mt * nt), dim3(WGM * WGN * 64), 0, stream.stream(), a, b, c,  \
          nullptr, M, N, K, lda, ldb, ldc, 0, mt, nt);                        \
    } else {                                                                  \
      hipLaunchKernelGGL(                                                     \
          (gemm_tr_kernel<BM, BN, FM, FN, MW, WGM, WGN, false, false, GM>),   \
          dim3(mt * nt), dim3(WGM * WGN * 64), 0, stream.stream(), a, b, c,  \
          nullptr, M, N, K, lda, ldb, ldc, 0, mt, nt);                        \
    }                                                                         \
  } while (0)
  switch (variant) {
    case 0: LV(128, 128, 2, 2, 4, 4, 4, 0); break;
    case 1: LV(128, 128, 2, 2, 4, 4, 4, 8); break;
    case 2: LV(64, 64, 2, 2, 6, 2, 2, 0); break;
    case 3: LV(64, 64, 2, 2, 6, 2, 2, 8); break;
    case 4: LV(256, 128, 4, 4, 2, 4, 2, 0); break;
    case 5: LV(128, 256, 4, 4, 2, 2, 4, 0); break;
    case 6: LV(128, 128, 2, 2, 4, 4, 4, 4); break;
    default: TORCH_CHECK(false, "unknown tr variant");
  }
#undef LV
  HIP_CHECK_KERNEL();
}

void gemm_tr_bf16(const at::Tensor& A, const at::Tensor& B, at::Tensor& C,
                  const c10::optional<at::Tensor>& bias, int64_t act,
                  int64_t trans_a, int64_t trans_b) {
  TORCH_CHECK(A.is_cuda() && B.is_cuda() && C.is_cuda(), "gemm_tr: GPU only");
  TORCH_CHECK(A.scalar_type() == at::kBFloat16 &&
                  B.scalar_type() == at::kBFloat16,
              "gemm_tr: bf16 required");
  const int M = (int)C.size(0), N = (int)C.size(1);
  const int K = (int)(trans_a ? A.size(0) : A.size(1));
  TORCH_CHECK((int)(trans_b ? B.size(0) : B.size(1)) == K, "K mismatch");
  TORCH_CHECK((int)(trans_a ? A.size(1) : A.size(0)) == M, "M mismatch");
  TORCH_CHECK((int)(trans_b ? B.size(1) : B.size(0)) == N, "N mismatch");
  const int lda = (int)A.stride(0), ldb = (int)B.stride(0),
            ldc = (int)C.stride(0);
  TORCH_CHECK(trans_a || trans_b,
              "gemm_tr: use gemm_nt_bf16 for the non-transposed case");
  TORCH_CHECK(K % 32 == 0 && lda % 8 == 0 && ldb % 8 == 0,
              "gemm_tr: fast-path alignment required "
              "(K%32, strides%8) — pad like HipLinear does");
  if (M == 0 || N == 0) return;
  const float* bias_ptr = nullptr;
  if (bias.has_value() && bias->defined()) bias_ptr = bias->data_ptr<float>();
  auto stream = at::cuda::getCurrentCUDAStream();
  const bf16_t* a = (const bf16_t*)A.data_ptr();
  const bf16_t* b = (const bf16_t*)B.data_ptr();
  bf16_t* c = (bf16_t*)C.data_ptr();
  const int64_t b128 = (int64_t)((M + 127) / 128) * ((N + 127) / 128);
  const int64_t t_256x128 = (int64_t)((M + 255) / 256) * ((N + 127) / 128);
  const int64_t t_128x256 = (int64_t)((M + 127) / 128) * ((N + 255) / 256);
  if (!trans_a && trans_b && K % 64 == 0 && b128 >= 256 && b128 < 1024) {
    gemm_x8(A, B, C, bias, act, trans_a, trans_b,
            b128 <= 256 ?  10 :  0);
    return;
  }
  if (trans_a && trans_b && K % 64 == 0 && b128 >= 256 && b128 < 1024) {
    gemm_x8(A, B, C, bias, act, trans_a, trans_b,  10);
    return;
  }
  const int64_t t256sq = (int64_t)((M + 255) / 256) * ((N + 255) / 256);
  if (trans_a && trans_b && K % 64 == 0 && t256sq >= 200) {
    gemm_x8(A, B, C, bias, act, trans_a, trans_b,  11);
    return;
  }
#define LTR(BM, BN, FM, FN, MW, WGM, WGN)                                     \
  do {                                                                        \
    const int mt = (M + BM - 1) / BM, nt = (N + BN - 1) / BN;                 \
    if (trans_a && trans_b) {                                                 \
      hipLaunchKernelGGL(                                                     \
          (gemm_tr_kernel<BM, BN, FM, FN, MW, WGM, WGN, true, true>),         \
          dim3(mt * nt), dim3(WGM * WGN * 64), 0, stream.stream(), a, b, c,  \
          bias_ptr, M, N, K, lda, ldb, ldc, (int)act, mt, nt);                \
    } else if (trans_b) {                                                     \
      hipLaunchKernelGGL(                                                     \
          (gemm_tr_kernel<BM, BN, FM, FN, MW, WGM, WGN, false, true>),        \
          dim3(mt * nt), dim3(WGM * WGN * 64), 0, stream.stream(), a, b, c,  \
          bias_ptr, M, N, K, lda, ldb, ldc, (int)act, mt, nt);                \
    } else {                                                                  \
      hipLaunchKernelGGL(                                                     \
          (gemm_tr_kernel<BM, BN, FM, FN, MW, WGM, WGN, true, false>),        \
          dim3(mt * nt), dim3(WGM * WGN * 64), 0, stream.stream(), a, b, c,  \
          bias_ptr, M, N, K, lda, ldb, ldc, (int)act, mt, nt);                \
    }                                                                         \
  } while (0)
  if (M <= 32 && N >= 256) {
    if (N >= 96) LTR(32, 128, 2, 4, 4, 1, 2);
    else LTR(32, 64, 2, 2, 4, 1, 2);
  } else if (M >= N && t_256x128 >= 512) {
    LTR(256, 128, 4, 4, 2, 4, 2);
  } else if (N > M && t_128x256 >= 512) {
    LTR(128, 256, 4, 4, 2, 2, 4);
  } else if (K >= M && K >= N && K <= 2048 && b128 >= 160 && b128 < 512) {
    LTR(64, 64, 2, 2, 6, 2, 2);
  } else if (b128 >= 160) {
    LTR(128, 128, 2, 2, 4, 4, 4);
  } else {
    LTR(64, 64, 2, 2, 6, 2, 2);
  }
#undef LTR
  HIP_CHECK_KERNEL();
}

void gemm_tr_batched(const at::Tensor& A, const at::Tensor& B, at::Tensor& C,
                     const c10::optional<at::Tensor>& bias, int64_t act,
                     int64_t trans_a, int64_t trans_b) {
  TORCH_CHECK(A.is_cuda() && B.is_cuda() && C.is_cuda(), "gemm_trb: GPU only");
  TORCH_CHECK(A.scalar_type() == at::kBFloat16 &&
                  B.scalar_type() == at::kBFloat16,
              "gemm_trb: bf16 required");
  TORCH_CHECK(C.dim() == 3, "gemm_trb: C must be [Z,M,N]");
  const int Z = (int)C.size(0);
  const int M = (int)C.size(1), N = (int)C.size(2);
  auto dims2 = [](const at::Tensor& t) {
    return std::make_pair((int)t.size(t.dim() - 2), (int)t.size(t.dim() - 1));
  };
  auto a2 = dims2(A), b2 = dims2(B);
  const int K = trans_a ? a2.first : a2.second;
  TORCH_CHECK((trans_b ? b2.second : b2.first) == N, "gemm_trb: N mismatch");
  TORCH_CHECK((trans_b ? b2.first : b2.second) == K, "gemm_trb: K mismatch");
  TORCH_CHECK((trans_a ? a2.second : a2.first) == M, "gemm_trb: M mismatch");
  const int lda = (int)A.stride(A.dim() - 2), ldb = (int)B.stride(B.dim() - 2),
            ldc = (int)C.stride(1);
  const int64_t sa = A.dim() == 3 ? A.stride(0) : 0;
  const int64_t sb = B.dim() == 3 ? B.stride(0) : 0;
  const int64_t sc = C.stride(0);
  TORCH_CHECK(K % 32 == 0 && lda % 8 == 0 && ldb % 8 == 0,
              "gemm_trb: fast-path alignment required (K%32, strides%8)");
  if (Z == 0 || M == 0 || N == 0) return;
  const float* bias_ptr = nullptr;
  if (bias.has_value() && bias->defined()) bias_ptr = bias->data_ptr<float>();
  auto stream = at::cuda::getCurrentCUDAStream();
  const bf16_t* a = (const bf16_t*)A.data_ptr();
  const bf16_t* b = (const bf16_t*)B.data_ptr();
  bf16_t* c = (bf16_t*)C.data_ptr();
#define LTRB(BM, BN, FM, FN, MW, WGM, WGN, TRA, TRB)                          \
  do {                                                                        \
    const int mt = (M + BM - 1) / BM, nt = (N + BN - 1) / BN;                 \
    hipLaunchKernelGGL(                                                       \
        (gemm_tr_kernel<BM, BN, FM, FN, MW, WGM, WGN, TRA, TRB>),             \
        dim3(mt * nt, 1, Z), dim3(WGM * WGN * 64), 0, stream.stream(), a, b, \
        c, bias_ptr, M, N, K, lda, ldb, ldc, (int)act, mt, nt, sa, sb, sc);   \
  } while (0)
#define LTRB_DISPATCH(TRA, TRB)                                               \
  do {                                                                        \
    const int64_t b128 = (int64_t)((M + 127) / 128) * ((N + 127) / 128);      \
    if (M <= 32) {                                                            \
         \
         \
         \
      if (N >= 96) LTRB(32, 128, 2, 4, 4, 1, 2, TRA, TRB);                    \
      else LTRB(32, 64, 2, 2, 4, 1, 2, TRA, TRB);                             \
    } else if (b128 >= 64) {                                                  \
      LTRB(128, 128, 2, 2, 4, 4, 4, TRA, TRB);                                \
    } else {                                                                  \
      LTRB(64, 64, 2, 2, 6, 2, 2, TRA, TRB);                                  \
    }                                                                         \
  } while (0)
  if (trans_a && trans_b) {
    LTRB_DISPATCH(true, true);
  } else if (trans_b) {
    LTRB_DISPATCH(false, true);
  } else if (trans_a) {
    LTRB_DISPATCH(true, false);
  } else {
    LTRB_DISPATCH(false, false);
  }
#undef LTRB
#undef LTRB_DISPATCH
  HIP_CHECK_KERNEL();
}
```

### adanet_amd/csrc/reduce.hip

```cpp

#include <torch/extension.h>
#include <ATen/cuda/CUDAContext.h>
#include "common.h"

__global__ __launch_bounds__(256) void colsum_bf16_kernel(
    const bf16_t* __restrict__ x, float* __restrict__ out, int B, int C,
    int ldx, int rows_per_block, int accum, float* __restrict__ wsp) {
  const int c = blockIdx.x * blockDim.x + threadIdx.x;
  if (c >= C) return;
  const int r0 = blockIdx.y * rows_per_block;
  const int r1 = min(B, r0 + rows_per_block);
  float acc = 0.f;
  for (int b = r0; b < r1; ++b) acc += bf2f(x[(int64_t)b * ldx + c]);
  if (gridDim.y == 1) {
    if (accum) out[c] += acc;
    else out[c] = acc;
  } else {
    wsp[(int64_t)blockIdx.y * C + c] = acc;
  }
}

__global__ __launch_bounds__(256) void colsum_reduce_kernel(
    const float* __restrict__ wsp, float* __restrict__ out, int C,
    int nchunks, int accum) {
  const int c = blockIdx.x * 4 + (threadIdx.x >> 6);
  if (c >= C) return;
  const float s = wave_slot_sum(wsp + c, C, nchunks);
  if ((threadIdx.x & 63) == 0) {
    if (accum) out[c] += s;
    else out[c] = s;
  }
}

void launch_colsum_reduce(const float* wsp, float* out, int C, int nchunks,
                          int accum, hipStream_t stream) {
  hipLaunchKernelGGL(colsum_reduce_kernel, dim3((unsigned)((C + 3) / 4)),
                     dim3(256), 0, stream, wsp, out, C, nchunks, accum);
}

__global__ __launch_bounds__(256) void argmax_correct_kernel(
    const bf16_t* __restrict__ logits, const int64_t* __restrict__ labels,
    int64_t* __restrict__ pred, int* __restrict__ correct, int B, int C,
    int ldl) {
  const int64_t stride = (int64_t)gridDim.x * blockDim.x;
  for (int64_t b = (int64_t)blockIdx.x * blockDim.x + threadIdx.x; b < B;
       b += stride) {
    const bf16_t* row = logits + b * ldl;
    float best = bf2f(row[0]);
    int arg = 0;
    for (int c = 1; c < C; ++c) {
      const float v = bf2f(row[c]);
      if (v > best) {
        best = v;
        arg = c;
      }
    }
    if (pred) pred[b] = arg;
    if (correct && arg == (int)labels[b]) atomicAdd(correct, 1);
  }
}

__global__ __launch_bounds__(256) void binary_histogram_kernel(
    const float* __restrict__ scores, const int64_t* __restrict__ labels,
    int* __restrict__ hist, int B, int T) {
  extern __shared__ int lh[];
  for (int i = threadIdx.x; i < 2 * T; i += blockDim.x) lh[i] = 0;
  __syncthreads();
  const int64_t stride = (int64_t)gridDim.x * blockDim.x;
  for (int64_t i = (int64_t)blockIdx.x * blockDim.x + threadIdx.x; i < B;
       i += stride) {
    float s = scores[i];
    s = s < 0.f ? 0.f : (s > 1.f ? 1.f : s);
    int b = (int)(s * T);
    b = b >= T ? T - 1 : b;
    atomicAdd(&lh[(labels[i] != 0 ? 0 : 1) * T + b], 1);
  }
  __syncthreads();
  for (int i = threadIdx.x; i < 2 * T; i += blockDim.x) {
    if (lh[i]) atomicAdd(&hist[i], lh[i]);
  }
}

void binary_histogram(const at::Tensor& scores, const at::Tensor& labels,
                      at::Tensor& hist) {
  TORCH_CHECK(scores.scalar_type() == at::kFloat && scores.is_contiguous(),
              "binary_histogram: contiguous fp32 scores");
  TORCH_CHECK(labels.scalar_type() == at::kLong, "binary_histogram: int64 labels");
  TORCH_CHECK(hist.scalar_type() == at::kInt && hist.dim() == 2 &&
                  hist.size(0) == 2,
              "binary_histogram: int32 [2,T] hist");
  const int B = (int)scores.numel(), T = (int)hist.size(1);
  if (B == 0) return;
  auto stream = at::cuda::getCurrentCUDAStream();
  const int blocks = std::min((B + 255) / 256, 512);
  hipLaunchKernelGGL(binary_histogram_kernel, dim3(blocks), dim3(256),
                     2 * T * sizeof(int), stream.stream(),
                     scores.data_ptr<float>(), labels.data_ptr<int64_t>(),
                     hist.data_ptr<int>(), B, T);
  HIP_CHECK_KERNEL();
}

void colsum_bf16(const at::Tensor& x, at::Tensor& out, int64_t accum) {
  const int B = (int)x.size(0), C = (int)x.size(1);
  if (C == 0) return;
  if (B == 0) { if (!accum) out.zero_(); return; }
  auto stream = at::cuda::getCurrentCUDAStream();
  const int stripes = (C + 255) / 256;
  int row_chunks = std::max(1, std::min(1024 / stripes, (B + 7) / 8));
  const int rows_per_block = (B + row_chunks - 1) / row_chunks;
  float* wsp = nullptr;
  at::Tensor wsp_t;
  if (row_chunks > 1) {
    wsp_t = at::empty({row_chunks, C}, out.options());
    wsp = wsp_t.data_ptr<float>();
  }
  hipLaunchKernelGGL(colsum_bf16_kernel,
                     dim3((unsigned)stripes, (unsigned)row_chunks), dim3(256),
                     0, stream.stream(), (const bf16_t*)x.data_ptr(),
                     out.data_ptr<float>(), B, C, (int)x.stride(0),
                     rows_per_block, (int)accum, wsp);
  if (wsp)
    launch_colsum_reduce(wsp, out.data_ptr<float>(), C, row_chunks,
                         (int)accum, stream.stream());
  HIP_CHECK_KERNEL();
}

void argmax_correct(const at::Tensor& logits, const at::Tensor& labels,
                    const c10::optional<at::Tensor>& pred,
                    at::Tensor& correct) {
  const int B = (int)logits.size(0), C = (int)logits.size(1);
  if (B == 0 || C == 0) return;
  auto stream = at::cuda::getCurrentCUDAStream();
  int64_t* pred_ptr =
      (pred && pred->defined()) ? pred->data_ptr<int64_t>() : nullptr;
  hipLaunchKernelGGL(argmax_correct_kernel,
                     dim3(std::min((B + 255) / 256, 2048)), dim3(256), 0,
                     stream.stream(), (const bf16_t*)logits.data_ptr(),
                     labels.data_ptr<int64_t>(), pred_ptr,
                     correct.data_ptr<int>(), B, C, (int)logits.stride(0));
  HIP_CHECK_KERNEL();
}
```

### adanet_amd/models/canned.py

```python

from __future__ import annotations

import functools
from typing import Callable, Optional, Sequence

import torch
from torch import nn

from adanet_amd.ops.dropout import HipDropout
from adanet_amd.ops.linear import HipLinear
from adanet_amd.ops.optim import FusedSGD
from adanet_amd.subnetwork.generator import SubnetworkModule


def _feature_dim(features) -> int:
    t = features
    if isinstance(features, dict):
        t = features[sorted(features.keys())[0]]
    return int(torch.tensor(t.shape[1:]).prod())


class _FlattenInput(nn.Module):

    def forward(self, features):
        x = features
        if isinstance(features, dict):
            x = features[sorted(features.keys())[0]]
        if x.dim() > 2:
            x = x.reshape(x.shape[0], -1)
        return x


class _LinearModule(SubnetworkModule):

    def __init__(self, in_dim, logits_dim):
        super().__init__()
        self.flatten = _FlattenInput()
        self.logits_layer = HipLinear(in_dim, logits_dim)
        self.last_layer_dim = in_dim

    def forward(self, features):
        x = self.flatten(features)
        return x, self.logits_layer(x)


class _DNNModule(SubnetworkModule):

    def __init__(self, in_dim, hidden_units, logits_dim, dropout):
        super().__init__()
        self.flatten = _FlattenInput()
        layers = []
        d = in_dim
        for h in hidden_units:
            layers.append(HipLinear(d, h, activation="relu"))
            if dropout:
                layers.append(HipDropout(dropout))
            d = h
        self.hidden = nn.Sequential(*layers)
        self.logits_layer = HipLinear(d, logits_dim)
        self.last_layer_dim = d

    def forward(self, features):
        x = self.flatten(features)
        last = self.hidden(x)
        return last, self.logits_layer(last)


class LinearEstimator(object):

    def __init__(self, head=None, optimizer: Optional[Callable] = None,
                 seed: Optional[int] = None):
        self.head = head
        self._optimizer = optimizer or functools.partial(FusedSGD, lr=0.01)
        self._seed = seed

    def build_model(self, features, logits_dimension, training):
        if self._seed is not None:
            torch.manual_seed(self._seed)
        return _LinearModule(_feature_dim(features), logits_dimension)

    def make_optimizer(self, params):
        return self._optimizer(params)


class DNNEstimator(object):

    def __init__(self, head=None, hidden_units: Sequence[int] = (300,),
                 optimizer: Optional[Callable] = None, dropout: float = 0.0,
                 seed: Optional[int] = None):
        self.head = head
        self.hidden_units = list(hidden_units)
        self._optimizer = optimizer or functools.partial(FusedSGD, lr=0.01)
        self.dropout = dropout
        self._seed = seed

    def build_model(self, features, logits_dimension, training):
        if self._seed is not None:
            torch.manual_seed(self._seed)
        return _DNNModule(_feature_dim(features), self.hidden_units,
                          logits_dimension, self.dropout if training else 0.0)

    def make_optimizer(self, params):
        return self._optimizer(params)


class _DNNLinearCombinedModule(SubnetworkModule):

    def __init__(self, in_dim, hidden_units, logits_dim, dropout):
        super().__init__()
        self.flatten = _FlattenInput()
        self.wide = HipLinear(in_dim, logits_dim)
        layers = []
        d = in_dim
        for h in hidden_units:
            layers.append(HipLinear(d, h, activation="relu"))
            if dropout:
                layers.append(HipDropout(dropout))
            d = h
        self.deep = nn.Sequential(*layers)
        self.deep_logits = HipLinear(d, logits_dim, bias=False)
        self.last_layer_dim = d

    def forward(self, features):
        x = self.flatten(features)
        last = self.deep(x)
        return last, self.wide(x) + self.deep_logits(last)


class DNNLinearCombinedEstimator(object):

    def __init__(self, head=None, hidden_units: Sequence[int] = (300,),
                 optimizer: Optional[Callable] = None,
                 linear_optimizer: Optional[Callable] = None,
                 dropout: float = 0.0, seed: Optional[int] = None):
        self.head = head
        self.hidden_units = list(hidden_units)
        self._optimizer = (optimizer or linear_optimizer
                           or functools.partial(FusedSGD, lr=0.01))
        self.dropout = dropout
        self._seed = seed

    def build_model(self, features, logits_dimension, training):
        if self._seed is not None:
            torch.manual_seed(self._seed)
        return _DNNLinearCombinedModule(
            _feature_dim(features), self.hidden_units, logits_dimension,
            self.dropout if training else 0.0)

    def make_optimizer(self, params):
        return self._optimizer(params)
```

### adanet_amd/models/simple_dnn.py

```python

from __future__ import annotations

import functools
from typing import List, Optional

import torch
from torch import nn

from adanet_amd.ops.dropout import HipDropout
from adanet_amd.ops.linear import HipLinear
from adanet_amd.ops.optim import FusedSGD
from adanet_amd.subnetwork.generator import (Builder, Generator, Subnetwork,
                                             SubnetworkModule)
from adanet_amd.subnetwork.report import Report


def _feature_dim(features) -> int:
    t = features
    if isinstance(features, dict):
        t = features[sorted(features.keys())[0]]
    return int(torch.tensor(t.shape[1:]).prod())


class _DNNModule(SubnetworkModule):

    def __init__(self, in_dim: int, num_layers: int, layer_size: int,
                 logits_dim: int, dropout: float):
        super().__init__()
        import os
        unfused = os.environ.get("ADANET_UNFUSED_DROPOUT", "") not in ("", "0")
        layers = []
        d = in_dim
        for _ in range(num_layers):
            layers.append(HipLinear(d, layer_size, activation="relu",
                                    dropout=0.0 if unfused else dropout))
            if unfused and dropout > 0:
                layers.append(HipDropout(dropout))
            d = layer_size
        self.hidden = nn.Sequential(*layers)
        self.logits_layer = HipLinear(d, logits_dim)
        self.last_layer_dim = d

    def forward(self, features):
        x = features
        if isinstance(features, dict):
            x = features[sorted(features.keys())[0]]
        if x.dim() > 2:
            x = x.reshape(x.shape[0], -1)
        last = self.hidden(x) if len(self.hidden) else x
        logits = self.logits_layer(last)
        return last, logits


class _SimpleDNNBuilder(Builder):

    def __init__(self, optimizer_fn, layer_size: int, num_layers: int,
                 learn_mixture_weights: bool, dropout: float, seed=None,
                 name_suffix: str = "", mixture_optimizer_fn=None):
        self._optimizer_fn = optimizer_fn
        self._mixture_optimizer_fn = mixture_optimizer_fn or optimizer_fn
        self._layer_size = layer_size
        self._num_layers = num_layers
        self._learn_mixture_weights = learn_mixture_weights
        self._dropout = dropout
        self._seed = seed
        self._name_suffix = name_suffix

    @property
    def name(self) -> str:
        base = ("linear" if self._num_layers == 0 else
                "{}_layer_dnn".format(self._num_layers))
        return base + self._name_suffix

    def build_subnetwork(self, features, logits_dimension, training,
                         previous_ensemble=None) -> Subnetwork:
        if self._seed is not None:
            suffix_code = sum(ord(c) * (i + 1)
                              for i, c in enumerate(self._name_suffix))
            torch.manual_seed(self._seed + self._num_layers * 7919 +
                              suffix_code)
        module = _DNNModule(_feature_dim(features), self._num_layers,
                            self._layer_size, logits_dimension,
                            self._dropout if training else 0.0)
        return Subnetwork(module=module,
                          complexity=float(self._num_layers ** 0.5),
                          shared={"num_layers": self._num_layers},
                          name=self.name)

    def build_optimizer(self, params, iteration: int = 0):
        return self._optimizer_fn(params)

    def build_mixture_weights_optimizer(self, params, iteration: int = 0):
        if not self._learn_mixture_weights:
            return None
        params = list(params)
        if not params:
            return None
        return self._mixture_optimizer_fn(params)

    def build_subnetwork_report(self) -> Report:
        return Report(hparams={"layer_size": self._layer_size,
                               "num_layers": self._num_layers},
                      attributes={"complexity": self._num_layers ** 0.5},
                      metrics={})


class Generator(Generator):

    def __init__(self, optimizer_fn=None, layer_size: int = 32,
                 initial_num_layers: int = 0,
                 learn_mixture_weights: bool = False, dropout: float = 0.0,
                 seed: Optional[int] = None, num_restarts: int = 1,
                 mixture_optimizer_fn=None):
        if optimizer_fn is None:
            optimizer_fn = functools.partial(FusedSGD, lr=0.01)
        self._builder_fn = functools.partial(
            _SimpleDNNBuilder,
            optimizer_fn=optimizer_fn,
            mixture_optimizer_fn=mixture_optimizer_fn,
            layer_size=layer_size,
            learn_mixture_weights=learn_mixture_weights,
            dropout=dropout,
            seed=seed)
        self._initial_num_layers = initial_num_layers
        self._num_restarts = max(1, int(num_restarts))

    def generate_candidates(self, previous_ensemble, iteration_number,
                            previous_ensemble_reports, all_reports,
                            config=None) -> List[Builder]:
        num_layers = self._initial_num_layers
        if previous_ensemble is not None:
            last = previous_ensemble.subnetworks[-1]
            shared = last.shared or {}
            num_layers = int(shared.get("num_layers",
                                        self._initial_num_layers))
        out = []
        for r in range(self._num_restarts):
            suffix = "" if r == 0 else "_r{}".format(r)
            out.append(self._builder_fn(num_layers=num_layers,
                                        name_suffix=suffix))
            out.append(self._builder_fn(num_layers=num_layers + 1,
                                        name_suffix=suffix))
        return out
```

### adanet_amd/ops/linear.py

```python

from __future__ import annotations

import math
from typing import Optional

import torch
from torch import nn

from adanet_amd.ops import _extension


_DIRECT_GRAD = False


class direct_grad_writes:

    def __enter__(self):
        global _DIRECT_GRAD
        self._prev = _DIRECT_GRAD
        _DIRECT_GRAD = True
        return self

    def __exit__(self, *exc):
        global _DIRECT_GRAD
        _DIRECT_GRAD = self._prev
        return False


def _pad8(n: int) -> int:
    return (n + 31) // 32 * 32


def restore_fp32_params(module) -> None:
    from adanet_amd.ops.conv import HipConv1x1, HipConvNxN
    from adanet_amd.ops.layernorm import HipLayerNorm
    for m in module.modules():
        if isinstance(m, (HipLinear, HipConv1x1, HipConvNxN)) \
                and m.bias is not None:
            m.bias.data = m.bias.data.float()
        if isinstance(m, HipLayerNorm) and m.weight is not None:
            m.weight.data = m.weight.data.float()
            m.bias.data = m.bias.data.float()
        from adanet_amd.ops.batchnorm import HipBatchNorm2d
        if isinstance(m, (torch.nn.modules.batchnorm._BatchNorm,
                          HipBatchNorm2d)):
            if m.weight is not None:
                m.weight.data = m.weight.data.float()
                m.bias.data = m.bias.data.float()
            if m.running_mean is not None:
                m.running_mean = m.running_mean.float()
                m.running_var = m.running_var.float()


def gemm_nt(a: torch.Tensor, b: torch.Tensor,
            bias: Optional[torch.Tensor] = None,
            activation: Optional[str] = None,
            dropout_p: float = 0.0,
            seed: Optional[torch.Tensor] = None) -> torch.Tensor:
    if a.is_cuda:
        ext = _extension.require()
        out = torch.empty((a.shape[0], b.shape[0]), device=a.device,
                          dtype=torch.bfloat16)
        if dropout_p > 0.0 and activation == "relu":
            ext.gemm_nt_bf16(a, b, out, bias, 3, dropout_p, seed)
        else:
            ext.gemm_nt_bf16(a, b, out, bias,
                             1 if activation == "relu" else 0)
        return out
    out = a.float() @ b.float().t()
    if bias is not None:
        out = out + bias.float()
    if activation == "relu":
        out = torch.relu(out)
    return out.to(a.dtype)


def transpose2d(x: torch.Tensor) -> torch.Tensor:
    if x.is_cuda:
        ext = _extension.require()
        out = torch.empty((x.shape[1], x.shape[0]), device=x.device,
                          dtype=x.dtype)
        ext.transpose_bf16(x, out)
        return out
    return x.t().contiguous()


class _LinearFn(torch.autograd.Function):

    @staticmethod
    def forward(ctx, x, weight, bias, activation, dropout_p=0.0, seed=None):
        x = x.contiguous()
        y = gemm_nt(x, weight, bias, activation, dropout_p, seed)
        ctx.activation = activation
        ctx.dropout_p = dropout_p
        ctx.has_bias = bias is not None
        ctx.param_refs = (weight if isinstance(weight, nn.Parameter) else None,
                          bias if isinstance(bias, nn.Parameter) else None)
        ctx.save_for_backward(x, weight, y if activation == "relu" else None)
        return y

    @staticmethod
    def backward(ctx, dy):
        x, weight, y = ctx.saved_tensors
        dy = dy.contiguous()
        need_dx = ctx.needs_input_grad[0]
        need_dw = ctx.needs_input_grad[1]
        if dy.is_cuda:
            ext = _extension.require()
            wparam, bparam = ctx.param_refs
            bg = bparam.grad if (_DIRECT_GRAD and bparam is not None) \
                else None
            direct_b = (ctx.has_bias and bg is not None and bg.is_cuda
                        and bg.dtype == torch.float32
                        and bg.shape == (dy.shape[1],)
                        and bg.is_contiguous())
            db_done = False
            if ctx.activation == "relu":
                scale = (1.0 / (1.0 - ctx.dropout_p)
                         if ctx.dropout_p > 0.0 else 1.0)
                dz = torch.empty_like(dy)
                if direct_b and dy.is_contiguous() and y.is_contiguous():
                    ext.relu_bwd_colsum(dy, y, dz, bg, scale)
                    db_done = True
                else:
                    ext.relu_bwd(dy, y, dz, scale)
            else:
                dz = dy
            dx = dw = None
            B, N = dz.shape
            K = weight.shape[1]
            if need_dx:
                if (weight.stride(0) % 8 == 0 and N % 32 == 0
                        and N <= max(B, K)):
                    dx = torch.empty((B, K), device=dz.device,
                                     dtype=torch.bfloat16)
                    ext.gemm_tr_bf16(dz, weight, dx, None, 0, 0, 1)
                else:
                    wt = transpose2d(weight)
                    dx = gemm_nt(dz, wt)
            if need_dw:
                wg = wparam.grad if (_DIRECT_GRAD and wparam is not None) \
                    else None
                direct_w = (wg is not None and wg.is_cuda
                            and wg.dtype == torch.bfloat16
                            and wg.shape == (N, K) and wg.is_contiguous())
                dw_out = wg if direct_w else torch.empty(
                    (N, K), device=dz.device, dtype=torch.bfloat16)
                if direct_w and getattr(wparam, "_adanet_grad_overwrite",
                                        False):
                    writes = getattr(wparam, "_adanet_bwd_writes", 0)
                    wparam._adanet_bwd_writes = writes + 1
                    epi = 0 if writes == 0 else 2
                else:
                    epi = 0 if not direct_w else 2
                if (B % 32 == 0 and dz.stride(0) % 8 == 0
                        and x.stride(0) % 8 == 0):
                    ext.gemm_tr_bf16(dz, x, dw_out, None, epi, 1, 1)
                else:
                    dzt = transpose2d(dz)
                    xt = transpose2d(x)
                    ext.gemm_nt_bf16(dzt, xt, dw_out, None, epi)
                dw = None if direct_w else dw_out
            db = None
            if ctx.has_bias and not db_done:
                if direct_b:
                    ext.colsum_bf16(dz, bg, 1)
                else:
                    db = torch.empty((dz.shape[1],), device=dz.device,
                                     dtype=torch.float32)
                    ext.colsum_bf16(dz, db)
        else:
            dzf = dy.float()
            if ctx.activation == "relu":
                dzf = dzf * (y > 0).float() if y is not None else dzf
                if ctx.dropout_p > 0.0:
                    dzf = dzf / (1.0 - ctx.dropout_p)
            dx = (dzf @ weight.float()).to(x.dtype) if need_dx else None
            dw = (dzf.t() @ x.float()).to(weight.dtype) if need_dw else None
            db = dzf.sum(dim=0) if ctx.has_bias else None
        return dx, dw, db, None, None, None


class HipLinear(nn.Module):

    def __init__(self, in_features: int, out_features: int, bias: bool = True,
                 activation: Optional[str] = None, device=None,
                 dtype: torch.dtype = torch.bfloat16,
                 dropout: float = 0.0):
        super().__init__()
        if activation not in (None, "relu"):
            raise ValueError("activation must be None or 'relu'")
        if dropout and activation != "relu":
            raise ValueError("fused dropout requires activation='relu'")
        if not 0.0 <= dropout < 1.0:
            raise ValueError("dropout must be in [0, 1)")
        self.in_features = in_features
        self.out_features = out_features
        self.padded_out = _pad8(out_features)
        self.activation = activation
        self.dropout = float(dropout)
        self.register_buffer("_drop_seed",
                             torch.zeros(1, dtype=torch.int64),
                             persistent=False)
        self.register_buffer("_drop_snap",
                             torch.zeros(1, dtype=torch.int64),
                             persistent=False)
        self._drop_seeded = False
        self.weight = nn.Parameter(
            torch.empty((self.padded_out, in_features), device=device,
                        dtype=dtype))
        self.weight._adanet_single_write = True
        if bias:
            self.bias = nn.Parameter(
                torch.zeros((self.padded_out,), device=device,
                            dtype=torch.float32))
        else:
            self.register_parameter("bias", None)
        self.reset_parameters()

    def reset_parameters(self):
        with torch.no_grad():
            bound = 1.0 / math.sqrt(self.in_features)
            self.weight.uniform_(-bound, bound)
            if self.padded_out != self.out_features:
                self.weight[self.out_features:].zero_()
            if self.bias is not None:
                self.bias.zero_()

    def forward(self, x):
        if x.dim() > 2:
            x = x.reshape(x.shape[0], -1)
        p = self.dropout if (self.training and self.dropout > 0.0) else 0.0
        if p > 0.0 and x.is_cuda:
            if not self._drop_seeded or self._drop_seed.device != x.device:
                base = int(torch.initial_seed()) & 0x7FFFFFFFFFFF
                self._drop_seed = torch.tensor(
                    [base + id(self) % 100003], dtype=torch.int64,
                    device=x.device)
                self._drop_snap = torch.zeros_like(self._drop_seed)
                self._drop_seeded = True
            self._drop_snap.copy_(self._drop_seed)
            self._drop_seed.add_(0x9E3779B9)
            snapshot = self._drop_snap
            y = _LinearFn.apply(x.to(self.weight.dtype), self.weight,
                                self.bias, self.activation, p, snapshot)
        else:
            y = _LinearFn.apply(x.to(self.weight.dtype), self.weight,
                                self.bias, self.activation)
            if p > 0.0:
                y = torch.nn.functional.dropout(y, p, training=True)
        if self.padded_out != self.out_features:
            y = y[:, :self.out_features]
        return y

    def extra_repr(self):
        return "in=%d, out=%d (padded %d), act=%s" % (
            self.in_features, self.out_features, self.padded_out,
            self.activation)
```

Baseline: 10360 iterations/hour.

## Fuse dense-stack backward with masked dX GEMM epilogue for ReLU

Adds a mask operand (act==4) to the GEMM kernels so the dX product of a layer is written already multiplied by the next layer's ReLU mask, taken from the saved activations. A new autograd function runs the whole hidden stack plus the logits layer as one op, and its backward chains these masked dX GEMMs. This is meant to remove the separate relu_bwd pass and its extra tensor read and write, plus the per-layer autograd overhead. The cost is an extra mask read in the GEMM epilogue, and the fused path only applies to dropout-free stacks whose shapes fit the fast routing.

```diff
diff --git a/adanet_amd/csrc/binding.cpp b/adanet_amd/csrc/binding.cpp
--- a/adanet_amd/csrc/binding.cpp
+++ b/adanet_amd/csrc/binding.cpp
@@ -11,13 +11,15 @@
               int64_t variant);
 void gemm_x8(const at::Tensor& A, const at::Tensor& B, at::Tensor& C,
              const c10::optional<at::Tensor>& bias, int64_t act,
-             int64_t trans_a, int64_t trans_b, int64_t variant);
+             int64_t trans_a, int64_t trans_b, int64_t variant,
+             const c10::optional<at::Tensor>& mask);
 void probe_tr16_layout(at::Tensor& out);
 void gemm_tr_probe(const at::Tensor& A, const at::Tensor& B, at::Tensor& C,
                    int64_t trans_a, int64_t trans_b, int64_t variant);
 void gemm_tr_bf16(const at::Tensor& A, const at::Tensor& B, at::Tensor& C,
                   const c10::optional<at::Tensor>& bias, int64_t act,
-                  int64_t trans_a, int64_t trans_b);
+                  int64_t trans_a, int64_t trans_b,
+                  const c10::optional<at::Tensor>& mask);
 void gemm_tr_batched(const at::Tensor& A, const at::Tensor& B, at::Tensor& C,
                      const c10::optional<at::Tensor>& bias, int64_t act,
                      int64_t trans_a, int64_t trans_b);
@@ -143,10 +145,18 @@
   m.def("gemm_nt8", &gemm_nt8,
         "8-phase deep-pipelined GEMM (256^2-class tiles)");
   m.def("gemm_x8", &gemm_x8,
-        "pipelined GEMM with K-major (transposed) operand staging");
+        "pipelined GEMM with K-major (transposed) operand staging",
+        py::arg("A"), py::arg("B"), py::arg("C"), py::arg("bias"),
+        py::arg("act"), py::arg("trans_a"), py::arg("trans_b"),
+        py::arg("variant"), py::arg("mask") = c10::nullopt);
   m.def("probe_tr16_layout", &probe_tr16_layout);
   m.def("gemm_tr_probe", &gemm_tr_probe);
-  m.def("gemm_tr_bf16", &gemm_tr_bf16);
+  m.def("gemm_tr_bf16", &gemm_tr_bf16,
+        "C = op(A) @ op(B)^T on K-major operands; act==4 with `mask` is the "
+        "dX epilogue C = mask > 0 ? A@B : +0 (trans_b only)",
+        py::arg("A"), py::arg("B"), py::arg("C"), py::arg("bias"),
+        py::arg("act"), py::arg("trans_a"), py::arg("trans_b"),
+        py::arg("mask") = c10::nullopt);
   m.def("gemm_tr_batched", &gemm_tr_batched);
   m.def("transpose_bf16", &transpose_bf16, "bf16 2-D transpose");
   m.def("softmax_xent_fwd", &softmax_xent_fwd);
diff --git a/adanet_amd/csrc/common.h b/adanet_amd/csrc/common.h
--- a/adanet_amd/csrc/common.h
+++ b/adanet_amd/csrc/common.h
@@ -69,6 +69,30 @@
 void launch_colsum_reduce(const float* wsp, float* out, int C, int nchunks,
                           int accum, hipStream_t stream);
 
+struct ColsumGeom {
+  int stripes, row_chunks, rows_per_block;
+};
+
+inline ColsumGeom colsum_geom(int B, int C) {
+  ColsumGeom g;
+  g.stripes = (C + 255) / 256;
+  const int want = 1024 / g.stripes, fit = (B + 7) / 8;
+  g.row_chunks = want < fit ? want : fit;
+  if (g.row_chunks < 1) g.row_chunks = 1;
+  g.rows_per_block = (B + g.row_chunks - 1) / g.row_chunks;
+  return g;
+}
+
+__device__ __forceinline__ void load_mask4(const bf16_t* __restrict__ mask,
+                                           int64_t ldm, int row_base, int M,
+                                           int col, float (&mv)[4]) {
+#pragma unroll
+  for (int rr = 0; rr < 4; ++rr) {
+    const int row = row_base + rr < M ? row_base + rr : M - 1;
+    mv[rr] = bf2f(mask[(int64_t)row * ldm + col]);
+  }
+}
+
 __device__ __forceinline__ uint32_t hash_rng(uint64_t seed, uint64_t idx) {
   uint64_t z = seed + 0x9e3779b97f4a7c15ull * (idx + 1);
   z = (z ^ (z >> 30)) * 0xbf58476d1ce4e5b9ull;
diff --git a/adanet_amd/csrc/elementwise.hip b/adanet_amd/csrc/elementwise.hip
--- a/adanet_amd/csrc/elementwise.hip
+++ b/adanet_amd/csrc/elementwise.hip
@@ -167,10 +167,9 @@
   const int B = (int)dy.size(0), C = (int)dy.size(1);
   if (B == 0 || C == 0) return;
   auto stream = at::cuda::getCurrentCUDAStream();
-  const int stripes = (C + 255) / 256;
-  const int row_chunks =
-      std::max(1, std::min(1024 / stripes, (B + 7) / 8));
-  const int rows_per_block = (B + row_chunks - 1) / row_chunks;
+  const ColsumGeom g = colsum_geom(B, C);
+  const int stripes = g.stripes, row_chunks = g.row_chunks;
+  const int rows_per_block = g.rows_per_block;
   auto wsp = at::empty({row_chunks, C}, db.options());
   hipLaunchKernelGGL(relu_bwd_colsum_kernel,
                      dim3((unsigned)stripes, (unsigned)row_chunks), dim3(256),
diff --git a/adanet_amd/csrc/gemm_8ph.hip b/adanet_amd/csrc/gemm_8ph.hip
--- a/adanet_amd/csrc/gemm_8ph.hip
+++ b/adanet_amd/csrc/gemm_8ph.hip
@@ -474,13 +474,15 @@
 
 template <int BM, int BN, int WN, bool TRA = false, bool TRB = false,
           bool BAR2 = false,
-          bool STAGGER = false>
+          bool STAGGER = false,
+          bool MASKED = false>
 __global__ __launch_bounds__(2 * WN * 64, 2) void gemm_ks_kernel(
     const bf16_t* __restrict__ A, const bf16_t* __restrict__ B,
     bf16_t* __restrict__ C, const float* __restrict__ bias, int M, int N,
     int K, int64_t lda, int64_t ldb, int64_t ldc, int act, int mtiles,
     int ntiles, const long long* __restrict__ seed = nullptr,
-    uint32_t pthresh = 0, float inv_keep = 1.f) {
+    uint32_t pthresh = 0, float inv_keep = 1.f,
+    const bf16_t* __restrict__ mask = nullptr, int64_t ldm = 0) {
   constexpr int NW = 2 * WN;
   constexpr int FM = BM / 32;
   constexpr int FN = BN / (WN * 16);
@@ -615,12 +617,17 @@
       const int col = col0 + wn * (FN * 16) + j * 16 + c_col_in_frag;
       if (col >= N) continue;
       const float bv = bias ? bias[col] : 0.f;
+      float mv[4];
+      if (MASKED)
+        load_mask4(mask, ldm, row0 + wm * (FM * 16) + i * 16 + c_row_base, M,
+                   col, mv);
 #pragma unroll
       for (int rr = 0; rr < 4; ++rr) {
         const int row = row0 + wm * (FM * 16) + i * 16 + c_row_base + rr;
         if (row >= M) continue;
         float v = acc[i][j][rr] + bv;
         if (act == 1) v = v > 0.f ? v : 0.f;
+        if (MASKED) v = mv[rr] > 0.f ? v : 0.f;
         if (act == 3) {
           v = v > 0.f ? v : 0.f;
           const uint32_t rnd =
@@ -715,12 +722,12 @@
   else if constexpr (N == 8) asm volatile("s_waitcnt lgkmcnt(8)" ::: "memory");
 }
 
-template <int BM, int BN, int WN, bool TRA, bool TRB>
+template <int BM, int BN, int WN, bool TRA, bool TRB, bool MASKED = false>
 __global__ __launch_bounds__(2 * WN * 64, 2) void gemm_x8_kernel(
     const bf16_t* __restrict__ A, const bf16_t* __restrict__ B,
     bf16_t* __restrict__ C, const float* __restrict__ bias, int M, int N,
     int K, int64_t lda, int64_t ldb, int64_t ldc, int act, int mtiles,
-    int ntiles) {
+    int ntiles, const bf16_t* __restrict__ mask = nullptr, int64_t ldm = 0) {
   constexpr int NW = 2 * WN;
   constexpr int FM = BM / (2 * 16);
   constexpr int FN = BN / (WN * 16);
@@ -899,12 +906,17 @@
       const int col = col0 + wn * (FN * 16) + j * 16 + c_col_in_frag;
       if (col >= N) continue;
       const float bv = bias ? bias[col] : 0.f;
+      float mv[4];
+      if (MASKED)
+        load_mask4(mask, ldm, row0 + wm * (FM * 16) + i * 16 + c_row_base, M,
+                   col, mv);
 #pragma unroll
       for (int rr = 0; rr < 4; ++rr) {
         const int row = row0 + wm * (FM * 16) + i * 16 + c_row_base + rr;
         if (row >= M) continue;
         float v = acc[i][j][rr] + bv;
         if (act == 1) v = v > 0.f ? v : 0.f;
+        if (MASKED) v = mv[rr] > 0.f ? v : 0.f;
         bf16_t* cp = &C[(int64_t)row * ldc + col];
         if (act == 2) v += bf2f(*cp);
         *cp = f2bf(v);
@@ -917,7 +929,8 @@
 
 void gemm_x8(const at::Tensor& A, const at::Tensor& B, at::Tensor& C,
              const c10::optional<at::Tensor>& bias, int64_t act,
-             int64_t trans_a, int64_t trans_b, int64_t variant) {
+             int64_t trans_a, int64_t trans_b, int64_t variant,
+             const c10::optional<at::Tensor>& mask) {
   const int M = (int)C.size(0), N = (int)C.size(1);
   const int K = (int)(trans_a ? A.size(0) : A.size(1));
   TORCH_CHECK((int)(trans_b ? B.size(1) : B.size(0)) == N &&
@@ -929,6 +942,25 @@
   TORCH_CHECK(lda % 8 == 0 && ldb % 8 == 0, "gemm_x8: 16B-aligned rows");
   const float* bias_ptr = nullptr;
   if (bias.has_value() && bias->defined()) bias_ptr = bias->data_ptr<float>();
+  const bool masked = mask.has_value() && mask->defined();
+  TORCH_CHECK(masked == (act == 4),
+              "gemm_x8: act==4 and the mask operand go together");
+  const bf16_t* mk = nullptr;
+  int64_t ldm = 0;
+  if (masked) {
+    TORCH_CHECK(bias_ptr == nullptr, "gemm_x8: act==4 takes no bias");
+    TORCH_CHECK(!trans_a && trans_b && (variant == 0 || variant == 10),
+                "gemm_x8: act==4 is trans_b-only, variants 0 and 10");
+    TORCH_CHECK(mask->is_cuda() && mask->scalar_type() == at::kBFloat16 &&
+                    mask->dim() == 2 && mask->size(0) == M &&
+                    mask->size(1) == N,
+                "gemm_x8: mask must be bf16 [M,N] on the GPU");
+    ldm = mask->stride(0);
+    TORCH_CHECK((N == 1 || mask->stride(1) == 1) && ldm % 8 == 0,
+                "gemm_x8: mask needs unit column stride and stride%8");
+    mk = (const bf16_t*)mask->data_ptr();
+  }
+  if (M == 0 || N == 0) return;
   auto stream = at::cuda::getCurrentCUDAStream();
   const bf16_t* a = (const bf16_t*)A.data_ptr();
   const bf16_t* b = (const bf16_t*)B.data_ptr();
@@ -948,6 +980,23 @@
     else if (trans_a) LX8(BM, BN, WNW, true, false);                          \
     else LX8(BM, BN, WNW, false, false);                                      \
   } while (0)
+  if (masked) {
+    const int mt = (M + 127) / 128, nt = (N + 127) / 128;
+    if (variant == 0) {
+      hipLaunchKernelGGL((gemm_x8_kernel<128, 128, 4, false, true, true>),
+                         dim3(mt * nt), dim3(512), 0, stream.stream(), a, b,
+                         c, bias_ptr, M, N, K, lda, ldb, ldc, (int)act, mt,
+                         nt, mk, ldm);
+    } else {
+      hipLaunchKernelGGL(
+          (gemm_ks_kernel<128, 128, 4, false, true, false, false, true>),
+          dim3(mt * nt), dim3(512), 0, stream.stream(), a, b, c, bias_ptr, M,
+          N, K, lda, ldb, ldc, (int)act, mt, nt,
+          (const long long*)nullptr, (uint32_t)0, 1.f, mk, ldm);
+    }
+    HIP_CHECK_KERNEL();
+    return;
+  }
   switch (variant) {
     case 0: LX8_T(128, 128, 4); break;
     case 1: LX8_T(128, 128, 2); break;
diff --git a/adanet_amd/csrc/gemm_tn.hip b/adanet_amd/csrc/gemm_tn.hip
--- a/adanet_amd/csrc/gemm_tn.hip
+++ b/adanet_amd/csrc/gemm_tn.hip
@@ -8,7 +8,8 @@
 
 void gemm_x8(const at::Tensor& A, const at::Tensor& B, at::Tensor& C,
              const c10::optional<at::Tensor>& bias, int64_t act,
-             int64_t trans_a, int64_t trans_b, int64_t variant);
+             int64_t trans_a, int64_t trans_b, int64_t variant,
+             const c10::optional<at::Tensor>& mask);
 
 typedef __attribute__((address_space(3))) const bf16_t* lds_cptr_t;
 
@@ -101,12 +102,13 @@
 }
 
 template <int BM, int BN, int FM, int FN, int MINWAVES, int WGM, int WGN,
-          bool TRA, bool TRB, int GROUPM = 0>
+          bool TRA, bool TRB, int GROUPM = 0, bool MASKED = false>
 __global__ __launch_bounds__(WGM * WGN * 64, MINWAVES) void gemm_tr_kernel(
     const bf16_t* __restrict__ A, const bf16_t* __restrict__ B,
     bf16_t* __restrict__ C, const float* __restrict__ bias, int M, int N,
     int K, int lda, int ldb, int ldc, int act, int mtiles, int ntiles,
-    int64_t stride_a = 0, int64_t stride_b = 0, int64_t stride_c = 0) {
+    int64_t stride_a = 0, int64_t stride_b = 0, int64_t stride_c = 0,
+    const bf16_t* __restrict__ mask = nullptr, int64_t ldm = 0) {
   constexpr int KSTEP = 32;
   __shared__ bf16_t As[2][BM * KSTEP];
   __shared__ bf16_t Bs[2][BN * KSTEP];
@@ -239,12 +241,17 @@
       const int col = col0 + wn * (FN * 16) + j * 16 + c_col_in_frag;
       if (col >= N) continue;
       const float bv = bias ? bias[col] : 0.f;
+      float mv[4];
+      if (MASKED)
+        load_mask4(mask, ldm, row0 + wm * (FM * 16) + i * 16 + c_row_base, M,
+                   col, mv);
 #pragma unroll
       for (int rr = 0; rr < 4; ++rr) {
         const int row = row0 + wm * (FM * 16) + i * 16 + c_row_base + rr;
         if (row >= M) continue;
         float v = acc[i][j][rr] + bv;
         if (act == 1) v = v > 0.f ? v : 0.f;
+        if (MASKED) v = mv[rr] > 0.f ? v : 0.f;
         bf16_t* cp = &C[(int64_t)row * ldc + col];
         if (act == 2) v += bf2f(*cp);
         *cp = f2bf(v);
@@ -301,7 +308,8 @@
 
 void gemm_tr_bf16(const at::Tensor& A, const at::Tensor& B, at::Tensor& C,
                   const c10::optional<at::Tensor>& bias, int64_t act,
-                  int64_t trans_a, int64_t trans_b) {
+                  int64_t trans_a, int64_t trans_b,
+                  const c10::optional<at::Tensor>& mask) {
   TORCH_CHECK(A.is_cuda() && B.is_cuda() && C.is_cuda(), "gemm_tr: GPU only");
   TORCH_CHECK(A.scalar_type() == at::kBFloat16 &&
                   B.scalar_type() == at::kBFloat16,
@@ -318,9 +326,27 @@
   TORCH_CHECK(K % 32 == 0 && lda % 8 == 0 && ldb % 8 == 0,
               "gemm_tr: fast-path alignment required "
               "(K%32, strides%8) — pad like HipLinear does");
+  const bool has_bias = bias.has_value() && bias->defined();
+  const bool masked = mask.has_value() && mask->defined();
+  TORCH_CHECK(masked == (act == 4),
+              "gemm_tr: act==4 and the mask operand go together");
+  const bf16_t* mk = nullptr;
+  int64_t ldm = 0;
+  if (masked) {
+    TORCH_CHECK(!has_bias, "gemm_tr: act==4 takes no bias");
+    TORCH_CHECK(!trans_a && trans_b, "gemm_tr: act==4 is trans_b-only (dX)");
+    TORCH_CHECK(mask->is_cuda() && mask->scalar_type() == at::kBFloat16,
+                "gemm_tr: bf16 GPU mask required");
+    TORCH_CHECK(mask->dim() == 2 && mask->size(0) == M && mask->size(1) == N,
+                "gemm_tr: mask must be [M,N]");
+    ldm = mask->stride(0);
+    TORCH_CHECK((N == 1 || mask->stride(1) == 1) && ldm % 8 == 0,
+                "gemm_tr: mask needs unit column stride and stride%8");
+    mk = (const bf16_t*)mask->data_ptr();
+  }
   if (M == 0 || N == 0) return;
   const float* bias_ptr = nullptr;
-  if (bias.has_value() && bias->defined()) bias_ptr = bias->data_ptr<float>();
+  if (has_bias) bias_ptr = bias->data_ptr<float>();
   auto stream = at::cuda::getCurrentCUDAStream();
   const bf16_t* a = (const bf16_t*)A.data_ptr();
   const bf16_t* b = (const bf16_t*)B.data_ptr();
@@ -330,16 +356,18 @@
   const int64_t t_128x256 = (int64_t)((M + 127) / 128) * ((N + 255) / 256);
   if (!trans_a && trans_b && K % 64 == 0 && b128 >= 256 && b128 < 1024) {
     gemm_x8(A, B, C, bias, act, trans_a, trans_b,
-            b128 <= 256 ?  10 :  0);
+            b128 <= 256 ?  10 :  0, mask);
     return;
   }
   if (trans_a && trans_b && K % 64 == 0 && b128 >= 256 && b128 < 1024) {
-    gemm_x8(A, B, C, bias, act, trans_a, trans_b,  10);
+    gemm_x8(A, B, C, bias, act, trans_a, trans_b,  10,
+            c10::nullopt);
     return;
   }
   const int64_t t256sq = (int64_t)((M + 255) / 256) * ((N + 255) / 256);
   if (trans_a && trans_b && K % 64 == 0 && t256sq >= 200) {
-    gemm_x8(A, B, C, bias, act, trans_a, trans_b,  11);
+    gemm_x8(A, B, C, bias, act, trans_a, trans_b,  11,
+            c10::nullopt);
     return;
   }
 #define LTR(BM, BN, FM, FN, MW, WGM, WGN)                                     \
@@ -350,6 +378,13 @@
           (gemm_tr_kernel<BM, BN, FM, FN, MW, WGM, WGN, true, true>),         \
           dim3(mt * nt), dim3(WGM * WGN * 64), 0, stream.stream(), a, b, c,  \
           bias_ptr, M, N, K, lda, ldb, ldc, (int)act, mt, nt);                \
+    } else if (trans_b && masked) {                                           \
+      hipLaunchKernelGGL(                                                     \
+          (gemm_tr_kernel<BM, BN, FM, FN, MW, WGM, WGN, false, true, 0,       \
+                          true>),                                             \
+          dim3(mt * nt), dim3(WGM * WGN * 64), 0, stream.stream(), a, b, c,  \
+          bias_ptr, M, N, K, lda, ldb, ldc, (int)act, mt, nt, (int64_t)0,     \
+          (int64_t)0, (int64_t)0, mk, ldm);                                   \
     } else if (trans_b) {                                                     \
       hipLaunchKernelGGL(                                                     \
           (gemm_tr_kernel<BM, BN, FM, FN, MW, WGM, WGN, false, true>),        \
diff --git a/adanet_amd/csrc/reduce.hip b/adanet_amd/csrc/reduce.hip
--- a/adanet_amd/csrc/reduce.hip
+++ b/adanet_amd/csrc/reduce.hip
@@ -105,9 +105,9 @@
   if (C == 0) return;
   if (B == 0) { if (!accum) out.zero_(); return; }
   auto stream = at::cuda::getCurrentCUDAStream();
-  const int stripes = (C + 255) / 256;
-  int row_chunks = std::max(1, std::min(1024 / stripes, (B + 7) / 8));
-  const int rows_per_block = (B + row_chunks - 1) / row_chunks;
+  const ColsumGeom g = colsum_geom(B, C);
+  const int stripes = g.stripes, row_chunks = g.row_chunks;
+  const int rows_per_block = g.rows_per_block;
   float* wsp = nullptr;
   at::Tensor wsp_t;
   if (row_chunks > 1) {
diff --git a/adanet_amd/models/canned.py b/adanet_amd/models/canned.py
--- a/adanet_amd/models/canned.py
+++ b/adanet_amd/models/canned.py
@@ -8,7 +8,7 @@
 from torch import nn
 
 from adanet_amd.ops.dropout import HipDropout
-from adanet_amd.ops.linear import HipLinear
+from adanet_amd.ops.linear import HipLinear, dense_stack
 from adanet_amd.ops.optim import FusedSGD
 from adanet_amd.subnetwork.generator import SubnetworkModule
 
@@ -62,8 +62,7 @@
 
     def forward(self, features):
         x = self.flatten(features)
-        last = self.hidden(x)
-        return last, self.logits_layer(last)
+        return dense_stack(x, self.hidden, self.logits_layer)
 
 
 class LinearEstimator(object):
diff --git a/adanet_amd/models/simple_dnn.py b/adanet_amd/models/simple_dnn.py
--- a/adanet_amd/models/simple_dnn.py
+++ b/adanet_amd/models/simple_dnn.py
@@ -8,7 +8,7 @@
 from torch import nn
 
 from adanet_amd.ops.dropout import HipDropout
-from adanet_amd.ops.linear import HipLinear
+from adanet_amd.ops.linear import HipLinear, dense_stack
 from adanet_amd.ops.optim import FusedSGD
 from adanet_amd.subnetwork.generator import (Builder, Generator, Subnetwork,
                                              SubnetworkModule)
@@ -47,9 +47,7 @@
             x = features[sorted(features.keys())[0]]
         if x.dim() > 2:
             x = x.reshape(x.shape[0], -1)
-        last = self.hidden(x) if len(self.hidden) else x
-        logits = self.logits_layer(last)
-        return last, logits
+        return dense_stack(x, self.hidden, self.logits_layer)
 
 
 class _SimpleDNNBuilder(Builder):
diff --git a/adanet_amd/ops/linear.py b/adanet_amd/ops/linear.py
--- a/adanet_amd/ops/linear.py
+++ b/adanet_amd/ops/linear.py
@@ -85,6 +85,90 @@
     return x.t().contiguous()
 
 
+def _tr_dx_route(weight: torch.Tensor, batch: int, n_out: int) -> bool:
+    return (weight.stride(0) % 8 == 0 and n_out % 32 == 0
+            and n_out <= max(batch, weight.shape[1]))
+
+
+def _bwd_dx(ext, dz, weight, mask=None):
+    B, N = dz.shape
+    K = weight.shape[1]
+    if _tr_dx_route(weight, B, N):
+        dx = torch.empty((B, K), device=dz.device, dtype=torch.bfloat16)
+        if mask is None:
+            ext.gemm_tr_bf16(dz, weight, dx, None, 0, 0, 1)
+        else:
+            ext.gemm_tr_bf16(dz, weight, dx, None, 4, 0, 1, mask)
+        return dx
+    if mask is not None:
+        raise RuntimeError("masked dX needs the transposed-staging route")
+    wt = transpose2d(weight)
+    return gemm_nt(dz, wt)
+
+
+def _bwd_dw(ext, dz, x, wparam):
+    B, N = dz.shape
+    K = x.shape[1]
+    wg = wparam.grad if (_DIRECT_GRAD and wparam is not None) else None
+    direct_w = (wg is not None and wg.is_cuda
+                and wg.dtype == torch.bfloat16
+                and wg.shape == (N, K) and wg.is_contiguous())
+    dw_out = wg if direct_w else torch.empty(
+        (N, K), device=dz.device, dtype=torch.bfloat16)
+    if direct_w and getattr(wparam, "_adanet_grad_overwrite", False):
+        writes = getattr(wparam, "_adanet_bwd_writes", 0)
+        wparam._adanet_bwd_writes = writes + 1
+        epi = 0 if writes == 0 else 2
+    else:
+        epi = 0 if not direct_w else 2
+    if B % 32 == 0 and dz.stride(0) % 8 == 0 and x.stride(0) % 8 == 0:
+        ext.gemm_tr_bf16(dz, x, dw_out, None, epi, 1, 1)
+    else:
+        dzt = transpose2d(dz)
+        xt = transpose2d(x)
+        ext.gemm_nt_bf16(dzt, xt, dw_out, None, epi)
+    return None if direct_w else dw_out
+
+
+def _direct_bias_grad(bparam, n_out: int):
+    bg = bparam.grad if (_DIRECT_GRAD and bparam is not None) else None
+    if (bg is not None and bg.is_cuda and bg.dtype == torch.float32
+            and bg.shape == (n_out,) and bg.is_contiguous()):
+        return bg
+    return None
+
+
+def _bwd_db(ext, dz, bg):
+    if bg is not None:
+        ext.colsum_bf16(dz, bg, 1)
+        return None
+    db = torch.empty((dz.shape[1],), device=dz.device, dtype=torch.float32)
+    ext.colsum_bf16(dz, db)
+    return db
+
+
+def _relu_bwd(ext, dy, y, bg, scale=1.0):
+    dz = torch.empty_like(dy)
+    if bg is not None and dy.is_contiguous() and y.is_contiguous():
+        ext.relu_bwd_colsum(dy, y, dz, bg, scale)
+        return dz, True
+    ext.relu_bwd(dy, y, dz, scale)
+    return dz, False
+
+
+def _cpu_layer_bwd(dy, x, weight, y, relu, dropout_p, need_dx, need_dw,
+                   has_bias):
+    dzf = dy.float()
+    if relu:
+        dzf = dzf * (y > 0).float() if y is not None else dzf
+        if dropout_p > 0.0:
+            dzf = dzf / (1.0 - dropout_p)
+    dx = (dzf @ weight.float()).to(x.dtype) if need_dx else None
+    dw = (dzf.t() @ x.float()).to(weight.dtype) if need_dw else None
+    db = dzf.sum(dim=0) if has_bias else None
+    return dx, dw, db
+
+
 class _LinearFn(torch.autograd.Function):
 
     @staticmethod
@@ -108,77 +192,153 @@
         if dy.is_cuda:
             ext = _extension.require()
             wparam, bparam = ctx.param_refs
-            bg = bparam.grad if (_DIRECT_GRAD and bparam is not None) \
-                else None
-            direct_b = (ctx.has_bias and bg is not None and bg.is_cuda
-                        and bg.dtype == torch.float32
-                        and bg.shape == (dy.shape[1],)
-                        and bg.is_contiguous())
+            bg = _direct_bias_grad(bparam, dy.shape[1]) \
+                if ctx.has_bias else None
             db_done = False
             if ctx.activation == "relu":
                 scale = (1.0 / (1.0 - ctx.dropout_p)
                          if ctx.dropout_p > 0.0 else 1.0)
-                dz = torch.empty_like(dy)
-                if direct_b and dy.is_contiguous() and y.is_contiguous():
-                    ext.relu_bwd_colsum(dy, y, dz, bg, scale)
-                    db_done = True
-                else:
-                    ext.relu_bwd(dy, y, dz, scale)
+                dz, db_done = _relu_bwd(ext, dy, y, bg, scale)
             else:
                 dz = dy
-            dx = dw = None
-            B, N = dz.shape
-            K = weight.shape[1]
-            if need_dx:
-                if (weight.stride(0) % 8 == 0 and N % 32 == 0
-                        and N <= max(B, K)):
-                    dx = torch.empty((B, K), device=dz.device,
-                                     dtype=torch.bfloat16)
-                    ext.gemm_tr_bf16(dz, weight, dx, None, 0, 0, 1)
-                else:
-                    wt = transpose2d(weight)
-                    dx = gemm_nt(dz, wt)
-            if need_dw:
-                wg = wparam.grad if (_DIRECT_GRAD and wparam is not None) \
-                    else None
-                direct_w = (wg is not None and wg.is_cuda
-                            and wg.dtype == torch.bfloat16
-                            and wg.shape == (N, K) and wg.is_contiguous())
-                dw_out = wg if direct_w else torch.empty(
-                    (N, K), device=dz.device, dtype=torch.bfloat16)
-                if direct_w and getattr(wparam, "_adanet_grad_overwrite",
-                                        False):
-                    writes = getattr(wparam, "_adanet_bwd_writes", 0)
-                    wparam._adanet_bwd_writes = writes + 1
-                    epi = 0 if writes == 0 else 2
-                else:
-                    epi = 0 if not direct_w else 2
-                if (B % 32 == 0 and dz.stride(0) % 8 == 0
-                        and x.stride(0) % 8 == 0):
-                    ext.gemm_tr_bf16(dz, x, dw_out, None, epi, 1, 1)
-                else:
-                    dzt = transpose2d(dz)
-                    xt = transpose2d(x)
-                    ext.gemm_nt_bf16(dzt, xt, dw_out, None, epi)
-                dw = None if direct_w else dw_out
+            dx = _bwd_dx(ext, dz, weight) if need_dx else None
+            dw = _bwd_dw(ext, dz, x, wparam) if need_dw else None
             db = None
             if ctx.has_bias and not db_done:
-                if direct_b:
-                    ext.colsum_bf16(dz, bg, 1)
+                db = _bwd_db(ext, dz, bg)
+        else:
+            dx, dw, db = _cpu_layer_bwd(
+                dy, x, weight, y, ctx.activation == "relu", ctx.dropout_p,
+                need_dx, need_dw, ctx.has_bias)
+        return dx, dw, db, None, None, None
+
+
+_FUSED_STACK = True
+stack_calls = {"fused": 0, "per_layer": 0}
+
+
+def set_fused_dense_stack(enabled: bool) -> bool:
+    global _FUSED_STACK
+    prev = _FUSED_STACK
+    _FUSED_STACK = bool(enabled)
+    return prev
+
+
+class _DenseStackFn(torch.autograd.Function):
+
+    @staticmethod
+    def forward(ctx, x, *params):
+        ctx.set_materialize_grads(False)
+        weights, biases = params[0::2], params[1::2]
+        h = x.contiguous()
+        acts = [h]
+        for w, b in zip(weights[:-1], biases[:-1]):
+            h = gemm_nt(h, w, b, "relu")
+            acts.append(h)
+        logits = gemm_nt(h, weights[-1], biases[-1], None)
+        ctx.param_refs = tuple(
+            p if isinstance(p, nn.Parameter) else None for p in params)
+        ctx.has_bias = tuple(b is not None for b in biases)
+        ctx.save_for_backward(*acts, *weights)
+        return h, logits
+
+    @staticmethod
+    def backward(ctx, g_last, g_logits):
+        n = len(ctx.has_bias)
+        acts = ctx.saved_tensors[:n]
+        weights = ctx.saved_tensors[n:]
+        grads = [None] * (1 + 2 * n)
+        cuda = acts[0].is_cuda
+        ext = _extension.require() if cuda else None
+        dz = g_logits.contiguous() if g_logits is not None else None
+        dy, extra = None, g_last
+        for l in range(n - 1, -1, -1):
+            relu = l < n - 1
+            x, weight = acts[l], weights[l]
+            if not relu and dz is None:
+                dy, extra = extra, None
+                continue
+            if dz is None and dy is None:
+                break
+            need_dx = l > 0 or ctx.needs_input_grad[0]
+            need_dw = ctx.needs_input_grad[1 + 2 * l]
+            has_bias = ctx.has_bias[l]
+            if cuda:
+                wparam = ctx.param_refs[2 * l]
+                bg = _direct_bias_grad(ctx.param_refs[2 * l + 1],
+                                       weight.shape[0]) if has_bias else None
+                db_done = False
+                if dz is None:
+                    dz, db_done = _relu_bwd(ext, dy.contiguous(),
+                                            acts[l + 1], bg)
+                db = _bwd_db(ext, dz, bg) if has_bias and not db_done \
+                    else None
+                dw = _bwd_dw(ext, dz, x, wparam) if need_dw else None
+                dx = None
+                if l == 0:
+                    dx = _bwd_dx(ext, dz, weight) if need_dx else None
+                    dz = dy = None
+                elif extra is not None:
+                    dy, dz = _bwd_dx(ext, dz, weight) + extra, None
                 else:
-                    db = torch.empty((dz.shape[1],), device=dz.device,
-                                     dtype=torch.float32)
-                    ext.colsum_bf16(dz, db)
-        else:
-            dzf = dy.float()
-            if ctx.activation == "relu":
-                dzf = dzf * (y > 0).float() if y is not None else dzf
-                if ctx.dropout_p > 0.0:
-                    dzf = dzf / (1.0 - ctx.dropout_p)
-            dx = (dzf @ weight.float()).to(x.dtype) if need_dx else None
-            dw = (dzf.t() @ x.float()).to(weight.dtype) if need_dw else None
-            db = dzf.sum(dim=0) if ctx.has_bias else None
-        return dx, dw, db, None, None, None
+                    dy, dz = None, _bwd_dx(ext, dz, weight, mask=x)
+            else:
+                gin = dz if not relu else dy
+                dx, dw, db = _cpu_layer_bwd(
+                    gin.contiguous(), x, weight,
+                    acts[l + 1] if relu else None, relu, 0.0, need_dx,
+                    need_dw, has_bias)
+                if extra is not None and dx is not None:
+                    dx = dx + extra
+                dy, dz = dx, None
+            extra = None
+            grads[1 + 2 * l] = dw
+            grads[2 + 2 * l] = db
+            if l == 0:
+                grads[0] = dx
+        return tuple(grads)
+
+
+def _stack_fusable(x, layers, logits_layer) -> bool:
+    if not _FUSED_STACK or not layers:
+        return False
+    if not isinstance(logits_layer, HipLinear) \
+            or logits_layer.activation is not None:
+        return False
+    for m in layers:
+        if not isinstance(m, HipLinear) or m.activation != "relu":
+            return False
+        if m.padded_out != m.out_features:
+            return False
+        if m.training and m.dropout > 0.0:
+            return False
+    if x.is_cuda:
+        B = x.shape[0]
+        for m in layers[1:] + [logits_layer]:
+            if m.weight.dtype != torch.bfloat16 or not _tr_dx_route(
+                    m.weight, B, m.padded_out):
+                return False
+    return True
+
+
+def dense_stack(x, hidden, logits_layer):
+    layers = list(hidden)
+    if x.dim() > 2:
+        x = x.reshape(x.shape[0], -1)
+    if not _stack_fusable(x, layers, logits_layer):
+        stack_calls["per_layer"] += 1
+        last = x
+        for m in layers:
+            last = m(last)
+        return last, logits_layer(last)
+    stack_calls["fused"] += 1
+    params = []
+    for m in layers + [logits_layer]:
+        params += [m.weight, m.bias]
+    last, logits = _DenseStackFn.apply(x.to(layers[0].weight.dtype), *params)
+    if logits_layer.padded_out != logits_layer.out_features:
+        logits = logits[:, :logits_layer.out_features]
+    return last, logits
 
 
 class HipLinear(nn.Module):
```

New measurement: 10580 iterations/hour, median of 6. 2.1% higher.
